# visinf/style-seqcvae

Hardware: AMD Instinct MI355X
Metric: captions/sec (train step) (higher is better)
Workload: dtype f32; 1 GPU; C2 train step: fwd+bwd+allreduce+clip+SGD, B=64/GPU, R=36, F=2048, L=20 (T=21), Z=128, V=10000, E=1000, H=1200, A=768, SENTIMENT_VAE=1; global_batch=64, parallelism=dp1

## Files before the change

include/ssc.h:

```cpp
#ifndef SSC_H
#define SSC_H

#include <stddef.h>
#include <stdint.h>

#ifdef __cplusplus
extern "C" {
#endif

#define SSC_OK 0
#define SSC_EINVAL (-1)
#define SSC_EALIGN (-2)
#define SSC_EHIP (-3)
#define SSC_EWORKSPACE (-4)

#define SSC_MAX_SEG 6

int ssc_version(void);
int ssc_last_hip_error(void);
const char* ssc_arch(void);

typedef struct {
  const float* A; const float* B;
  int lda, ldb, K;
  const void* A16; const void* B16;
  int lda16, ldb16;
} ssc_gemm_seg;

typedef struct {
  ssc_gemm_seg seg[SSC_MAX_SEG];
  int nseg;
  int M, N;
  int a_kc, b_kc;
  float* C; int ldc;
  const float* bias;
  int accumulate;
  int splits;
  float* workspace; size_t workspace_floats;
  const int* m_count; const int* a_rows; const int* c_rows;
  const int* k_count; const int* ka_rows; const int* kb_rows;
  const float* a_scale; const float* b_scale;
  float* topk_part;
} ssc_gemm_desc;

int ssc_pow2_scale(const float* x, size_t rows, int cols, size_t ld, int target_log2, float* out, int combine, float* scratch,
                   void* stream);

int ssc_split_f16(const float* x, int rows, int K, int ldx, const float* scale, void* out, int ldo, const int* row_list,
                  const int* row_count, void* stream);

int ssc_gemm(const ssc_gemm_desc* d, void* stream);

int ssc_gemm_dw_group(const ssc_gemm_desc* const* d, int n, void* stream);

int ssc_set_gemm_mode(int mode);
int ssc_gemm_auto_splits(int M, int N, int ksteps);

int ssc_feat_prep(const float* feats, int B, int R, int F, float* mask, float* avg, void* stream);

int ssc_prep_tokens(const int64_t* caps, int B, int L, int pad, int boundary, int64_t* tokens_tm, float* w_tm,
                    float* nvalid, void* stream);

int ssc_embed_gather(const float* table, int ldt, const int64_t* ids, int n, int E, float* out, int ldo, void* stream);
int ssc_embed_scatter_add(float* dtable, int ldt, const int64_t* ids, int n, int E, const float* d, int ldd, int pad,
                          void* stream);

typedef struct {
  int B, H;
  const float* slabs; int nslab; size_t slab_stride;
  const float* add0; int ld_add0;
  const float* add1; int ld_add1; int rows_per_add1;
  const float* b_ih; const float* b_hh;
  const float* sent; const float* wcol; int ldwcol;
  const float* c_prev; int ld_cprev;
  float* gates_out;
  float* c_out; int ld_cout;
  float* h_out; int ld_hout;
  const int64_t* add0_rows;
  const int* slab_rows;
  const float* slabs2; int nslab2; size_t slab2_stride; const int* slab2_rows;
  const int* c_prev_rows;
  const int* rows; const int* row_count;
  void* h_planes; int ld_hplanes; const float* planes_scale;
} ssc_lstm_fwd_desc;
int ssc_lstm_fwd(const ssc_lstm_fwd_desc* d, void* stream);
int ssc_lstm_fwd_z(const ssc_lstm_fwd_desc* d, const float* z, int ldz, const float* wz, int ldwz, int Z, void* stream);
int ssc_lstm_fwd_p(const ssc_lstm_fwd_desc* d, const float* wp, int ldwp, int NP, float* pout, void* stream);
int ssc_lstm_fwd_img(const ssc_lstm_fwd_desc* d, const float* alpha, int ldalpha, const float* P, int R, int rows_per_image,
                     void* stream);

typedef struct {
  int B, H;
  const float* dh; int ld_dh;
  const float* dh2; int ld_dh2;
  const float* dc_in; int ld_dcin;
  const float* gates;
  const float* c_prev; int ld_cprev;
  const float* c_new; int ld_cnew;
  float* dG;
  float* dc_prev; int ld_dcprev;
  float* dgsum;
  const float* slabsA; int nA; size_t strideA;
  const float* slabsB; int nB; size_t strideB;
} ssc_lstm_bwd_desc;
int ssc_lstm_bwd(const ssc_lstm_bwd_desc* d, void* stream);
int ssc_lstm_bwd_x(const ssc_lstm_bwd_desc* d, const float* x, int ldx, const float* w, int ldw, int K, void* stream);

int ssc_attn_logits(const float* q, int ldq, const float* pv, const float* wa, int G, int R, int A, int rows_per_image,
                    float* logits, void* stream);
int ssc_attn_fwd(const float* q, int ldq, const float* pv, const float* wa, const float* mask, const float* feats,
                 int G, int R, int A, int F, int rows_per_image, float* logits, float* alpha, float* att, int ldatt,
                 void* stream);

int ssc_attn_weights(const float* q, int ldq, const float* pv, const float* wa, const float* mask, int G, int R, int A,
                     int rows_per_image, float* logits, float* alpha, void* stream);

int ssc_attn_pool(const float* alpha, const float* x, int G, int R, int D, int rows_per_image, float* out, int ldo,
                  void* stream);
int ssc_attn_fwd_pool(const float* q, int ldq, const float* pv, const float* wa, const float* mask, const float* feats,
                      int G, int R, int A, int F, int rows_per_image, float* logits, float* alpha, float* att, int ldatt,
                      const float* obj, int D, float* pool, int ldpool, void* stream);

int ssc_attn_bwd(const float* datt, int lddatt, const float* q, int ldq, const float* pv, const float* wa,
                 const float* alpha, const float* feats, int G, int R, int A, int F, float* dq, int lddq,
                 float* dpv_acc, float* dwa_acc, float* scratch_dalpha, void* stream);
int ssc_attn_bwd_pool(const float* datt, int lddatt, const float* q, int ldq, const float* pv, const float* wa,
                      const float* alpha, const float* feats, int G, int R, int A, int F, float* dq, int lddq,
                      float* dpv_acc, float* dwa_acc, float* scratch_dalpha, const float* obj, int D, const float* dpool_a,
                      int lddpa, int Da, const float* dpool_b, int lddpb, void* stream);

typedef struct {
  int B, Z;
  const float* mulv; int ldmulv; int nslab; size_t slab_stride;
  const float* bmu; const float* blv;
  const float* eps; int ldeps;
  int kld_mode;
  const float* sent; float pm_scale; float prior_var;
  const float* w;
  float* mu; float* lv; float* z; int ldz;
  float* kld_acc;
  const float* pm; int ldpm;
} ssc_latent_fwd_desc;
int ssc_latent_fwd(const ssc_latent_fwd_desc* d, void* stream);

// ... 472 lines not shown
```

style-seqcvae_amd/csrc/gemm.hip:

```cpp
#include <stdio.h>
#include <stdlib.h>
#include <string.h>

#include "ssc_common.h"
#include "ssc_debug.h"

typedef float f32x16 __attribute__((ext_vector_type(16)));

namespace {

constexpr int BM = 64, BN = 64, BK = 32;
constexpr int KC_LD = BK + 4;

struct KSeg {
  const float* A;
  const float* B;
  int lda, ldb, K, nsteps;
  int avec, bvec;
  const float* A16;
  const float* B16;
  int lda16, ldb16;
};

struct KArgs {
  KSeg seg[SSC_MAX_SEG];
  int nseg;
  int M, N;
  float* out;
  int ldo;
  size_t slab_stride;
  const float* bias;
  int accumulate;
  int steps_total, steps_per_split;
  const int* mcount;
  const int* arows;
  const int* crows;
  const int* kcount;
  const int* karows;
  const int* kbrows;
  int tile_gm;
  int store_wt;
  int member;
  float* topk;
  const float* a_scale;
  const float* b_scale;
};

__device__ __forceinline__ void tile_order(int lin, int gx, int gy, int gm, int& bx, int& by) {
  const int total = gx * gy;
  const int q = total >> 3, rem = total & 7;
  const int xcd = lin & 7, slot = lin >> 3;
  const int nl = xcd * q + (xcd < rem ? xcd : rem) + slot;
  if (gm <= 1 || gy <= 1) {
    by = nl / gx;
    bx = nl - by * gx;
    return;
  }
  const int group_sz = gm * gx;
  const int g = nl / group_sz;
  const int first_row = g * gm;
  const int rows = min(gy - first_row, gm);
  const int r = nl - g * group_sz;
  bx = r / rows;
  by = first_row + (r - bx * rows);
}

template <bool KC, int ROWS, bool VEC>
__device__ __forceinline__ unsigned load_tile(float (&r)[ROWS / 8], const float* __restrict__ base, int ld, int rows, int K,
                                              int row0, int k0, int tid) {
  constexpr int NV = ROWS / 32;
  unsigned okm = 0;
  if constexpr (KC && VEC) {
#pragma unroll
    for (int u = 0; u < NV; ++u) {
      int idx = tid + 256 * u;
      int row = idx >> 3, kq = idx & 7;
      int grow = min(row0 + row, rows - 1), k = k0 + 4 * kq;
      float4 v = *reinterpret_cast<const float4*>(base + (size_t)grow * ld + min(k, K - 4));
      okm |= (k < K ? 1u : 0u) << u;
      r[4 * u] = v.x; r[4 * u + 1] = v.y; r[4 * u + 2] = v.z; r[4 * u + 3] = v.w;
    }
  } else if constexpr (KC && !VEC) {
#pragma unroll
    for (int u = 0; u < 4 * NV; ++u) {
      int idx = tid + 256 * u;
// ... 765 lines not shown
      SSC_X3B_MFMA(0, 2)
      SSC_X3B_MFMA(1, 1)
      SSC_X3B_MFMA(1, 0)
      SSC_X3B_MFMA(0, 1)
      SSC_X3B_MFMA(0, 0)
#undef SSC_X3B_MFMA
    }
  };

  for (int s = s_lo; s < s_hi; ++s) {
    compute();
    wait_loads();
    __syncthreads();
    if (s + 1 < s_hi) put_planes();
    advance();
    issue_loads();
    __syncthreads();
  }
  wait_loads();

  float* out = a.out + (size_t)z * a.slab_stride;
#pragma unroll
  for (int ni = 0; ni < 2; ++ni) {
    const int col = n0 + wn * 64 + ni * 32 + l31;
    if (col >= a.N) continue;
    const float bv = (a.bias != nullptr) ? a.bias[col] : 0.f;
#pragma unroll
    for (int mi = 0; mi < 2; ++mi) {
      const int rbase = m0 + wm * 64 + mi * 32 + 4 * half;
      int rr[16];
#pragma unroll
      for (int r = 0; r < 16; ++r) {
        rr[r] = min(rbase + (r & 3) + 8 * (r >> 2), Meff - 1);
        if (a.crows) rr[r] = a.crows[rr[r]];
      }
      float old[16];
      if (a.accumulate) {
#pragma unroll
        for (int r = 0; r < 16; ++r) old[r] = out[(size_t)rr[r] * a.ldo + col];
      } else {
#pragma unroll
        for (int r = 0; r < 16; ++r) old[r] = 0.f;
      }
#pragma unroll
      for (int r = 0; r < 16; ++r) {
        if (rbase + (r & 3) + 8 * (r >> 2) < Meff) out[(size_t)rr[r] * a.ldo + col] = acc[mi][ni][r] + bv + old[r];
      }
    }
  }
}


#ifdef SSC_X3W_STAMP
__device__ unsigned long long* g_stamp_ptr = nullptr;
__device__ int g_stamp_wg = -1;
#define SSC_STAMP(i)                                                                                  \
  do {                                                                                                \
    if (stamp_on && lane == 0 && (i) < 124) stamp_lds[(i)] = __builtin_readcyclecounter();           \
  } while (0)
constexpr int X3W_STAMP_BYTES = 2048;
#else
#define SSC_STAMP(i) do {} while (0)
constexpr int X3W_STAMP_BYTES = 0;
#endif
#ifdef SSC_X3W_AUDIT
constexpr int SSC_AUDIT_MEMBERS = 20;
__device__ long long g_audit[SSC_AUDIT_MEMBERS][SSC_MAX_SEG][2][2];
#define SSC_AUDIT_TOUCH(member, seg, op, off)                                       \
  do {                                                                              \
    atomicMin(&g_audit[(member)][(seg)][(op)][0], (long long)(off));                \
    atomicMax(&g_audit[(member)][(seg)][(op)][1], (long long)(off) + 16);           \
  } while (0)
#else
#define SSC_AUDIT_TOUCH(member, seg, op, off) do {} while (0)
#endif
template <int R> struct X3wPlane {
  static constexpr int MC_ROW_B = 2 * R + 64;
  static constexpr int KC_BYTES = R * PL_ROW_B, MC_BYTES = 32 * MC_ROW_B;
  static constexpr int BYTES = KC_BYTES > MC_BYTES ? KC_BYTES : MC_BYTES;
};
template <int TM, int TN> constexpr int x3w_lds_bytes() { return 2 * 3 * (X3wPlane<TM>::BYTES + X3wPlane<TN>::BYTES) + X3W_STAMP_BYTES; }
template <int TM, int TN> constexpr int x3w_lds_bytes_f16() { return 2 * 2 * (X3wPlane<TM>::BYTES + X3wPlane<TN>::BYTES) + X3W_STAMP_BYTES; }

template <bool A_KC, bool B_KC, bool KG, int TM, int TN, int PF, int NPW, bool F16 = false, class Args = KArgs>
__device__ __forceinline__ void x3w_body(const Args& a, const int blk_x, const int blk_y, const int blk_z, const int grid_x,
                                         const int grid_y, const int grid_z, const int thr) {
  static_assert((TM == 128 && TN == 128) || (TM == 64 && TN == 256), "unsupported tile");
  static_assert(PF == 1 || PF == 2, "prefetch depth");
  constexpr int UNR = 2;
  constexpr bool RL = TM == 128;
  static_assert(!KG || PF == 1, "the gather lists' own loads share the vector-memory counter");
  constexpr int NPL = F16 ? 2 : 3;
  constexpr int PLA = X3wPlane<TM>::BYTES, PLB = X3wPlane<TN>::BYTES, STAGE = NPL * (PLA + PLB);
  static_assert(TM * (TN + 4) * 4 <= 2 * STAGE, "the epilogue's C tile reuses the operand stages");
  constexpr int MCA = X3wPlane<TM>::MC_ROW_B, MCB = X3wPlane<TN>::MC_ROW_B;
  static_assert(NPW == 4 || NPW == 8, "producer waves");
  constexpr int NPT = 64 * NPW;
  constexpr int NTHR = 256 + NPT;
  constexpr int NA = TM * 8 / NPT, NB = TN * 8 / NPT;
  constexpr int QA = TM / 4, QB = TN / 4;
  auto kc_row = [&](int t, int u, int) __attribute__((always_inline)) -> int { return (t + NPT * u) >> 3; };
  extern __shared__ __attribute__((aligned(16))) unsigned char lds[];
  const int wave = thr >> 6;
  const bool producer = wave >= 4;
  const int tid = producer ? thr - 256 : thr;
  const int lane = tid & 63;
  int bx, by;
  const int Meff = (RL && a.mcount) ? min(a.M, *a.mcount) : a.M;
  const int gy_live = min(grid_y, (Meff + TM - 1) / TM);
  if (blk_y * grid_x + blk_x >= grid_x * gy_live) return;
  tile_order(blk_y * grid_x + blk_x, grid_x, gy_live, a.tile_gm, bx, by);
  const int n0 = bx * TN, m0 = by * TM, z = blk_z;
  if (m0 >= Meff) return;
  const int Kc = a.kcount ? max(0, min(a.seg[0].K, *a.kcount)) : 0;
  int steps_total = a.steps_total, steps_per_split = a.steps_per_split;
  if (a.kcount) {
    steps_total = (Kc + BK - 1) / BK;
    steps_per_split = (steps_total + grid_z - 1) / grid_z;
  }
  const int s_lo = z * steps_per_split;
  int s_hi = s_lo + steps_per_split;
  if (s_hi > steps_total) s_hi = steps_total;
  const int s_last = s_hi - 1;
  constexpr int CT_LD = TN + 4;
  float f16_sa = 1.f, f16_sb = 1.f;
  if constexpr (F16) {
    if (a.a_scale) f16_sa = *a.a_scale;
    if (a.b_scale) f16_sb = *a.b_scale;
  }
#ifdef SSC_X3W_STAMP
  const bool stamp_on = (int)blockIdx.x == g_stamp_wg && (wave == 0 || wave == 4);
  unsigned long long* stamp_lds = reinterpret_cast<unsigned long long*>(lds + 2 * STAGE) + (wave == 4 ? 0 : 128);
  if (stamp_on && lane == 0) { stamp_lds[126] = __builtin_readcyclecounter(); stamp_lds[127] = wall_clock64(); }
  const unsigned long long stamp_entry = wall_clock64();
#endif

  if (producer) {
    f32x4 ra[PF][NA], rb[PF][NB];
    unsigned oka[PF], okb[PF];
    bool fullk[PF];
    unsigned oa[NA], ob[NB];
    unsigned za[NA], zb[NB];
    int ia[2][NA], ib[2][NB];
    Cursor cur;
    int s_ld = s_lo;
    bool pa = false, pb = false;
    auto planes_of_segment = [&]() __attribute__((always_inline)) {
      if constexpr (F16) {
        const KSeg& sg = a.seg[cur.seg];
        pa = sg.A16 != nullptr; pb = sg.B16 != nullptr;
        if (pa) { cur.A = sg.A16; cur.lda = sg.lda16; }
        if (pb) { cur.B = sg.B16; cur.ldb = sg.ldb16; }
      }
    };
    auto base_ptrs = [&]() __attribute__((always_inline)) {
      const unsigned lda4 = (unsigned)cur.lda * 4u, ldb4 = (unsigned)cur.ldb * 4u;
#pragma unroll
      for (int u = 0; u < NA; ++u) {
        const int idx = tid + NPT * u;
        if constexpr (A_KC) {
          int r = min(m0 + kc_row(tid, u, NA), Meff - 1);
          if constexpr (RL) { if (a.arows) r = a.arows[r]; }
          za[u] = (unsigned)r * lda4;
          oa[u] = za[u] + 16u * (idx & 7);
        } else {
          za[u] = 4u * (unsigned)min(m0 + 4 * (idx % QA), Meff - 4);
// ... 326 lines not shown
        float mx = -INFINITY, v0 = -INFINITY, v1 = -INFINITY;
        int i0 = -1, i1 = -1;
        const float inv = F16 ? 1.0f / (f16_sa * f16_sb) : 1.0f;
        float x[32];
        const bool wide_b = a.bias && !(reinterpret_cast<uintptr_t>(a.bias) & 15) && n0 + TN <= a.N;
#pragma unroll
        for (int j = 0; j < 8; ++j) {
          const float4 c4 = *reinterpret_cast<const float4*>(&ct[row * CT_LD + part * 32 + 4 * j]);
          float4 b4 = make_float4(0.f, 0.f, 0.f, 0.f);
          const int gc = n0 + part * 32 + 4 * j;
          if (wide_b) b4 = *reinterpret_cast<const float4*>(a.bias + gc);
          else if (a.bias) { b4.x = gc < a.N ? a.bias[gc] : 0.f; b4.y = gc + 1 < a.N ? a.bias[gc + 1] : 0.f; b4.z = gc + 2 < a.N ? a.bias[gc + 2] : 0.f; b4.w = gc + 3 < a.N ? a.bias[gc + 3] : 0.f; }
          x[4 * j] = c4.x * inv + b4.x; x[4 * j + 1] = c4.y * inv + b4.y; x[4 * j + 2] = c4.z * inv + b4.z; x[4 * j + 3] = c4.w * inv + b4.w;
        }
#pragma unroll
        for (int j = 0; j < 32; ++j) {
          const int gcol = n0 + part * 32 + j;
          if (gcol < a.N) {
            mx = fmaxf(mx, x[j]);
            if (x[j] > v0) { v1 = v0; i1 = i0; v0 = x[j]; i0 = gcol; }
            else if (x[j] > v1) { v1 = x[j]; i1 = gcol; }
          }
        }
#pragma unroll
        for (int o = 1; o <= 2; o <<= 1) mx = fmaxf(mx, __shfl_xor(mx, o, 64));
        float se = 0.f;
#pragma unroll
        for (int j = 0; j < 32; ++j) {
          const int gcol = n0 + part * 32 + j;
          if (gcol < a.N) se += __builtin_amdgcn_exp2f((x[j] - mx) * 1.4426950408889634f);
        }
#pragma unroll
        for (int o = 1; o <= 2; o <<= 1) se += __shfl_xor(se, o, 64);
#pragma unroll
        for (int o = 1; o <= 2; o <<= 1) {
          const float w0 = __shfl_xor(v0, o, 64), w1 = __shfl_xor(v1, o, 64);
          const int j0 = __shfl_xor(i0, o, 64), j1 = __shfl_xor(i1, o, 64);
          auto before = [](float xa, int ia, float xb, int ib) { return ib < 0 || (ia >= 0 && (xa > xb || (xa == xb && ia < ib))); };
          float r0, r1; int k0, k1;
          if (before(v0, i0, w0, j0)) {
            r0 = v0; k0 = i0;
            if (before(v1, i1, w0, j0)) { r1 = v1; k1 = i1; } else { r1 = w0; k1 = j0; }
          } else {
            r0 = w0; k0 = j0;
            if (before(v0, i0, w1, j1)) { r1 = v0; k1 = i0; } else { r1 = w1; k1 = j1; }
          }
          v0 = r0; i0 = k0; v1 = r1; i1 = k1;
        }
        if (part == 0 && grow < Meff) {
          const int rr = (RL && a.crows) ? a.crows[grow] : grow;
          float* rec = a.topk + ((size_t)rr * ntn + bx) * 6;
          rec[0] = mx; rec[1] = se; rec[2] = v0; rec[3] = __int_as_float(i0); rec[4] = v1; rec[5] = __int_as_float(i1);
        }
      }
      return;
    }
  }
  {
    const float* ct = reinterpret_cast<const float*>(lds);
    float* out = a.out + (size_t)z * a.slab_stride;
    const bool wide = !(a.ldo & 3) && !(a.N & 3) && !(a.slab_stride & 3) && !(reinterpret_cast<uintptr_t>(a.out) & 15) &&
                      !(reinterpret_cast<uintptr_t>(a.bias) & 15);
    constexpr int CPR = TN / 4;
#pragma unroll
    for (int i = 0; i < (TM * CPR + NTHR - 1) / NTHR; ++i) {
      const int c = thr + NTHR * i;
      if (TM * CPR % NTHR != 0 && c >= TM * CPR) break;
      const int row = c / CPR, col = 4 * (c % CPR);
      const int grow = m0 + row, gcol = n0 + col;
      if (grow >= Meff || gcol >= a.N) continue;
      const int rr = (RL && a.crows) ? a.crows[grow] : grow;
      float4 v = *reinterpret_cast<const float4*>(&ct[row * CT_LD + col]);
      if constexpr (F16) { const float inv = 1.0f / (f16_sa * f16_sb); v.x *= inv; v.y *= inv; v.z *= inv; v.w *= inv; }
      float* dst = out + (size_t)rr * a.ldo + gcol;
      if (wide) {
        if (a.bias) { const float4 b4 = *reinterpret_cast<const float4*>(a.bias + gcol); v.x += b4.x; v.y += b4.y; v.z += b4.z; v.w += b4.w; }
        if (a.accumulate) { const float4 o4 = *reinterpret_cast<const float4*>(dst); v.x += o4.x; v.y += o4.y; v.z += o4.z; v.w += o4.w; }
        if (a.store_wt) {
          const f32x4 v4 = {v.x, v.y, v.z, v.w};
          asm volatile("global_store_dwordx4 %0, %1, off sc1" ::"v"(dst), "v"(v4) : "memory");
        } else {
          *reinterpret_cast<float4*>(dst) = v;
        }
      } else {
        const float e[4] = {v.x, v.y, v.z, v.w};
#pragma unroll
        for (int q = 0; q < 4; ++q) {
          if (gcol + q < a.N) dst[q] = e[q] + (a.bias ? a.bias[gcol + q] : 0.f) + (a.accumulate ? dst[q] : 0.f);
        }
      }
    }
  }
#ifdef SSC_X3W_STAMP
  if (stamp_on && lane == 0) { stamp_lds[124] = __builtin_readcyclecounter(); stamp_lds[125] = wall_clock64(); }
  __syncthreads();
  if ((int)blockIdx.x == g_stamp_wg && thr < 256 && g_stamp_ptr)
    g_stamp_ptr[thr] = reinterpret_cast<const unsigned long long*>(lds + 2 * STAGE)[thr];
  if (g_stamp_wg == -2 && thr == 0 && g_stamp_ptr && blockIdx.x < 1024) {
    g_stamp_ptr[2 * blockIdx.x] = stamp_entry;
    g_stamp_ptr[2 * blockIdx.x + 1] = wall_clock64();
  }
#endif
}


constexpr int SSC_GROUP_MAX = 6;
struct KGroup {
  KArgs a[SSC_GROUP_MAX];
  int n;
  int first[SSC_GROUP_MAX + 1];
  int gx[SSC_GROUP_MAX], gy[SSC_GROUP_MAX], gz[SSC_GROUP_MAX];
};
template <bool A_KC, bool B_KC, bool KG, int TM, int TN, int PF, int NPW, bool F16 = false>
__global__ __launch_bounds__(256 + 64 * NPW, (F16 && NPW == 4) ? 4 : 1) void gemm_x3w_kernel(const KGroup g) {
  const int w = blockIdx.x;
  int p = 0;
#pragma unroll
  for (int i = 1; i < SSC_GROUP_MAX; ++i)
    if (i < g.n && w >= g.first[i]) p = i;
  const int local = w - g.first[p];
  const int gx = g.gx[p], gy = g.gy[p], gz = g.gz[p];
  const int x = local % gx, yz = local / gx;
  x3w_body<A_KC, B_KC, KG, TM, TN, PF, NPW, F16>(g.a[p], x, yz % gy, yz / gy, gx, gy, gz, (int)threadIdx.x);
}

constexpr int SSC_DW_MAX = 20;
struct KTnMember {
  const float* A;
  const float* B;
  float* C;
  const int* kcount;
  const int* karows;
  const int* kbrows;
  int lda, ldb, ldc, M, N, K, accumulate;
  int first;
};
struct KTnList {
  KTnMember m[SSC_DW_MAX];
  int n, total;
  int tile_gm, store_wt;
};
struct KOneSeg {
  KSeg s;
  __device__ __forceinline__ const KSeg& operator[](int) const { return s; }
};
struct KTnArgs {
  KOneSeg seg;
  int nseg, M, N;
  float* out;
  int ldo;
  size_t slab_stride;
  const float* bias;
  int accumulate, steps_total, steps_per_split;
  const int *mcount, *arows, *crows, *kcount, *karows, *kbrows;
  int tile_gm, store_wt, member;
  float* topk;
  const float *a_scale, *b_scale;
};
template <int PF, int NPW>
__global__ __launch_bounds__(256 + 64 * NPW, 1) void gemm_x3w_kernel_tn_list(const KTnList g) {
  int p = 0;
  for (int t = blockIdx.x; t < g.total; t += gridDim.x) {
#pragma unroll 1
    while (p + 1 < g.n && t >= g.m[p + 1].first) ++p;
    const KTnMember& m = g.m[p];
    int thr = (int)threadIdx.x;
    asm volatile("" : "+v"(thr));
    __builtin_assume(thr >= 0 && thr < 256 + 64 * NPW);
    KTnArgs a;
    a.seg.s.A = m.A; a.seg.s.B = m.B; a.seg.s.lda = m.lda; a.seg.s.ldb = m.ldb; a.seg.s.K = m.K;
    a.seg.s.nsteps = (m.K + BK - 1) / BK; a.seg.s.avec = a.seg.s.bvec = 1;
    a.seg.s.A16 = a.seg.s.B16 = nullptr; a.seg.s.lda16 = a.seg.s.ldb16 = 0;
    a.nseg = 1; a.M = m.M; a.N = m.N;
    a.out = m.C; a.ldo = m.ldc; a.slab_stride = 0; a.bias = nullptr; a.accumulate = m.accumulate;
    a.steps_total = a.steps_per_split = a.seg.s.nsteps;
    a.mcount = a.arows = a.crows = nullptr;
    a.kcount = m.kcount; a.karows = m.karows; a.kbrows = m.kbrows;
    a.tile_gm = g.tile_gm; a.store_wt = g.store_wt; a.member = p;
    a.topk = nullptr; a.a_scale = a.b_scale = nullptr;
    const int gx = (m.N + 127) / 128, gy = (m.M + 127) / 128;
    const int local = t - m.first;
    x3w_body<false, false, true, 128, 128, PF, NPW>(a, local % gx, local / gx, 0, gx, gy, 1, thr);
    __syncthreads();
  }
}

__global__ void reduce_slabs_kernel(const float* __restrict__ slabs, int nslab, size_t slab_stride, int M, int N,
                                    float* __restrict__ C, int ldc, const float* __restrict__ bias, int accumulate,
                                    const int* __restrict__ mcount, const int* __restrict__ crows) {
  size_t i = (size_t)blockIdx.x * blockDim.x + threadIdx.x;
  if (mcount) M = min(M, *mcount);
  size_t total = (size_t)M * N;
  if (i >= total) return;
  int row = (int)(i / N), col = (int)(i % N);
  float v = 0.f;
  for (int s0 = 0; s0 < nslab; s0 += 8) {
    float t[8];
#pragma unroll
    for (int u = 0; u < 8; ++u) t[u] = slabs[(size_t)min(s0 + u, nslab - 1) * slab_stride + i];
#pragma unroll
    for (int u = 0; u < 8; ++u) v += (s0 + u < nslab) ? t[u] : 0.f;
  }
  if (bias) v += bias[col];
  if (crows) row = crows[row];
  float* p = C + (size_t)row * ldc + col;
  if (accumulate) v += *p;
  *p = v;
}

typedef void (*gemm_fn)(const KArgs);

struct ProfMember { int M, N, K, slot_m, slot_k; };
struct ProfRec {
  hipEvent_t e0, e1;
  int kind, M, N, K, splits;
  double bytes, flops;
  ProfMember mem[8];
  int nmem;
};
int* g_prof_counts = nullptr;
int g_prof_slots = 0;
constexpr int PROF_SLOTS = 8192;
inline int prof_count_slot(const int* dev_count, hipStream_t st) {
  if (!dev_count || !g_prof_counts || g_prof_slots >= PROF_SLOTS) return -1;
  const int slot = g_prof_slots++;
  g_prof_counts[slot] = -1;
  if (hipMemcpyAsync(&g_prof_counts[slot], dev_count, sizeof(int), hipMemcpyDeviceToHost, st) != hipSuccess) return -1;
  return slot;
}
inline void prof_desc(ProfRec* rec, const ssc_gemm_desc* d, hipStream_t st) {
  int K = 0;
  for (int i = 0; i < d->nseg; ++i) K += d->seg[i].K;
  if (rec->nmem < 8) {
    ProfMember& m = rec->mem[rec->nmem++];
    m.M = d->M; m.N = d->N; m.K = K;
    m.slot_m = prof_count_slot(d->m_count, st);
    m.slot_k = prof_count_slot(d->k_count, st);
  }
}
constexpr int PROF_MAX = 4096;
ProfRec* g_prof = nullptr;
int g_prof_n = 0;
bool g_prof_on = false;

int g_store_wt = ssc_env_int("SSC_STORE_WT", 1);
int g_tile_gm = ssc_env_int("SSC_TILE_GM", 8);
int build_args(const ssc_gemm_desc* d, KArgs& k) {
  if (!d || d->nseg < 1 || d->nseg > SSC_MAX_SEG || d->M <= 0 || d->N <= 0) return SSC_EINVAL;
  k.tile_gm = g_tile_gm;
  k.store_wt = g_store_wt;
  k.member = 0;
  k.nseg = d->nseg;
  k.M = d->M;
  k.N = d->N;
  k.mcount = d->m_count; k.arows = d->a_rows; k.crows = d->c_rows;
  k.kcount = d->k_count; k.karows = d->ka_rows; k.kbrows = d->kb_rows;
  k.a_scale = d->a_scale; k.b_scale = d->b_scale;
  k.topk = d->topk_part;
  k.steps_total = 0;
  for (int i = 0; i < d->nseg; ++i) {
    const ssc_gemm_seg& s = d->seg[i];
    if (!s.A || !s.B || s.K <= 0) return SSC_EINVAL;
// ... 384 lines not shown
  KGroup g;
  bool ok = n >= 2, any_wide = false;
  long work = 0;
  const bool mid = d[0] && d[0]->M > 64 && d[0]->M >= BIG_MIN_M;
  const int tw = mid ? 128 : 256;
  for (int i = 0; i < n && ok; ++i) {
    SSC_TRY(build_args(d[i], g.a[i]));
    const KArgs& k = g.a[i];
    const bool compact = k.mcount || k.arows || k.crows || k.kcount || k.karows || k.kbrows;
    const bool shape = mid ? g_x3b != 0 && g_x3b != 3 && d[i]->M >= BIG_MIN_M && d[i]->M < 512 && d[i]->M == d[0]->M
                           : x3w_skinny_layout(d[i]) && d[i]->M <= 64;
    ok = !compact && x3w_ok(d[i], k, num) && d[i]->a_kc && shape && d[i]->N >= 64 && d[i]->b_kc == d[0]->b_kc && regions[i];
    any_wide = any_wide || (mid ? big_tile(d[i]->M, d[i]->N) : d[i]->N >= X3W_MIN_N);
    work += (long)ssc_cdiv(d[i]->N, tw) * ssc_cdiv(d[i]->M, mid ? 128 : 64) * k.steps_total;
  }
  ok = ok && any_wide;
  if (!ok) {
    for (int i = 0; i < n; ++i) SSC_TRY(ssc_gemm_slabs_auto(d[i], regions[i], caps[i], &nslab[i], st));
    return SSC_OK;
  }
  int per = (int)((work + 255) / 256);
  if (per < 4) per = 4;
  for (;; ++per) {
    long wgs = 0;
    for (int i = 0; i < n; ++i) wgs += (long)ssc_cdiv(d[i]->N, tw) * ssc_cdiv(d[i]->M, mid ? 128 : 64) * ssc_cdiv(g.a[i].steps_total, per);
    if (wgs <= 256 || per >= 4096) break;
  }
  g.n = n;
  g.first[0] = 0;
  int Ksum = 0, Nmax = 0;
  for (int i = 0; i < n; ++i) {
    KArgs& k = g.a[i];
    k.member = i;
    const size_t mn = (size_t)d[i]->M * d[i]->N;
    int splits = ssc_cdiv(k.steps_total, per);
    const int cap = (int)(caps[i] / mn);
    if (cap < 1) return SSC_EWORKSPACE;
    if (splits > cap) splits = cap;
    const int p2 = ssc_cdiv(k.steps_total, splits);
    splits = ssc_cdiv(k.steps_total, p2);
    k.steps_per_split = p2;
    k.out = regions[i];
    k.ldo = d[i]->N;
    k.slab_stride = mn;
    k.bias = nullptr;
    k.accumulate = 0;
    k.crows = nullptr;
    g.gx[i] = ssc_cdiv(d[i]->N, tw);
    g.gy[i] = mid ? ssc_cdiv(d[i]->M, 128) : 1;
    g.gz[i] = splits;
    g.first[i + 1] = g.first[i] + g.gx[i] * g.gy[i] * splits;
    nslab[i] = splits;
    for (int s = 0; s < d[i]->nseg; ++s) Ksum += d[i]->seg[s].K;
    if (d[i]->N > Nmax) Nmax = d[i]->N;
  }
  for (int i = n; i < SSC_GROUP_MAX; ++i) { g.first[i + 1] = g.first[n]; g.gx[i] = 1; g.gy[i] = 1; g.gz[i] = 1; }
  ProfRec* rec = prof_open(d, n, d[0]->M, Nmax, Ksum, nslab[0], st);
  if (mid) return launch_x3w(x3w_big(true, d[0]->b_kc != 0, false), g, true, d[0]->b_kc != 0, "128x128 group", rec, st);
  return launch_x3w(x3w_skinny_form(d[0]->b_kc != 0), g, true, d[0]->b_kc != 0, "64x256 group", rec, st);
}

namespace {
int launch_tn_list(const ssc_gemm_desc* const* d, const KArgs* ka, int n, hipStream_t st) {
  SSC_TRY(x3w_prepare());
  int dev = 0;
  if (hipGetDevice(&dev) != hipSuccess) return SSC_EHIP;
  int ord[SSC_DW_MAX];
  for (int i = 0; i < n; ++i) ord[i] = i;
  for (int i = 1; i < n; ++i)
    for (int j = i; j > 0 && ka[ord[j]].steps_total > ka[ord[j - 1]].steps_total; --j) { const int t = ord[j]; ord[j] = ord[j - 1]; ord[j - 1] = t; }
  KTnList g;
  memset(&g, 0, sizeof(g));
  const ssc_gemm_desc* ds[SSC_DW_MAX];
  KArgs audit[SSC_DW_MAX];
  int first = 0;
  long MN = 0;
  for (int i = 0; i < n; ++i) {
    const ssc_gemm_desc* di = d[ord[i]];
    KTnMember& m = g.m[i];
    m.A = di->seg[0].A; m.B = di->seg[0].B; m.C = di->C;
    m.kcount = di->k_count; m.karows = di->ka_rows; m.kbrows = di->kb_rows;
    m.lda = di->seg[0].lda; m.ldb = di->seg[0].ldb; m.ldc = di->ldc;
    m.M = di->M; m.N = di->N; m.K = di->seg[0].K; m.accumulate = di->accumulate;
    m.first = first;
    first += ssc_cdiv(di->M, 128) * ssc_cdiv(di->N, 128);
    MN += (long)di->M * di->N;
    ds[i] = di;
    audit[i] = ka[ord[i]];
    audit[i].out = di->C; audit[i].ldo = di->ldc;
  }
  g.n = n; g.total = first;
  g.tile_gm = g_tile_gm; g.store_wt = g_store_wt;
  ProfRec* rec = prof_open(ds, n, (int)(MN / ds[0]->N), ds[0]->N, ds[0]->seg[0].K, 1, st);
  SSC_AUDIT_BEGIN();
  SSC_LAUNCH(g_tn_list_fn, dim3(first < g_cus[dev] ? first : g_cus[dev]), dim3(TN_LIST_THREADS), TN_LIST_LDS, st, g);
  SSC_AUDIT_END(audit, n, false, false, "128x128 TN list", st);
  (void)audit;
  prof_close(rec, st);
  SSC_CHECK_LAUNCH();
  return SSC_OK;
}
}
extern "C" int ssc_gemm_dw_group(const ssc_gemm_desc* const* d, int n, void* stream) {
  hipStream_t st = (hipStream_t)stream;
  constexpr int NMAX = 32;
  if (!d || n < 1 || n > NMAX) return SSC_EINVAL;
  const Num num = numerics();
  KArgs ka[NMAX];
  int cls[NMAX];
  for (int j = 0; j < n; ++j) {
    const ssc_gemm_desc* dj = d[j];
    KArgs& k = ka[j];
    SSC_TRY(build_args(dj, k));
    const bool kg = k.karows || k.kbrows;
    const bool ok = x3w_ok(dj, k, num) && k.nseg == 1 && !dj->a_kc && !dj->b_kc && dj->C && dj->ldc >= dj->N && !k.mcount &&
                    !k.arows && !k.crows && (kg ? (k.kcount && k.karows && k.kbrows && !dj->bias) : !k.kcount);
    cls[j] = !ok ? 0 : kg ? 2 : 1;
  }
  const ssc_gemm_desc* ld[SSC_DW_MAX];
  KArgs lk[SSC_DW_MAX];
  int ln = 0;
  for (int j = 0; j < n; ++j) {
    if (cls[j] != 2) continue;
    ld[ln] = d[j]; lk[ln] = ka[j];
    if (++ln == SSC_DW_MAX) { SSC_TRY(launch_tn_list(ld, lk, ln, st)); ln = 0; }
  }
  if (ln) SSC_TRY(launch_tn_list(ld, lk, ln, st));
  int i = 0;
  while (i < n) {
    if (cls[i] == 2) { ++i; continue; }
    int m = 0;
    while (cls[i] == 1 && i + m < n && cls[i + m] == 1 && m < SSC_GROUP_MAX) ++m;
    if (m >= 2) {
      KGroup g;
      g.n = m;
      g.first[0] = 0;
      long MN = 0;
      for (int q = 0; q < m; ++q) {
        const ssc_gemm_desc* dj = d[i + q];
        KArgs& k = g.a[q];
        k = ka[i + q];
        k.member = q;
        k.steps_per_split = k.steps_total;
        k.out = dj->C; k.ldo = dj->ldc; k.slab_stride = 0; k.bias = dj->bias; k.accumulate = dj->accumulate;
        g.gx[q] = ssc_cdiv(dj->N, 128); g.gy[q] = ssc_cdiv(dj->M, 128); g.gz[q] = 1;
        g.first[q + 1] = g.first[q] + g.gx[q] * g.gy[q];
        MN += (long)dj->M * dj->N;
      }
      for (int q = m; q < SSC_GROUP_MAX; ++q) { g.first[q + 1] = g.first[m]; g.gx[q] = g.gy[q] = g.gz[q] = 1; }
      ProfRec* rec = prof_open(d + i, m, (int)(MN / d[i]->N), d[i]->N, d[i + m - 1]->seg[0].K, 1, st);
      SSC_TRY(launch_x3w(x3w_big(false, false, false), g, false, false, "128x128 TN group", rec, st));
      i += m;
    } else {
      SSC_TRY(ssc_gemm(d[i], (void*)st));
      ++i;
    }
  }
  return SSC_OK;
}

namespace {
__global__ __launch_bounds__(256) void split_f16_kernel(const float* __restrict__ x, int rows, int K, int ldx, const float* __restrict__ scale,
                                                        unsigned* __restrict__ out, int ldo, const int* __restrict__ row_list,
                                                        const int* __restrict__ row_count) {
  const int kq = blockIdx.x * blockDim.x + threadIdx.x;
  const int kp4 = (K + BK - 1) / BK * (BK / 4);
  if (kq >= kp4) return;
  const float sc = scale ? *scale : 1.f;
  const int n = row_list ? min(rows, *row_count) : rows;
  const bool vec = !(ldx & 3) && ssc_aligned16_dev(x);
  const int k = 4 * kq;
  for (int i = blockIdx.y; i < n; i += gridDim.y) {
    const int r = row_list ? row_list[i] : i;
    const float* xr = x + (size_t)r * ldx;
    f32x4 v;
    if (k + 4 <= K && vec) v = *reinterpret_cast<const f32x4*>(xr + k);
    else
#pragma unroll
      for (int j = 0; j < 4; ++j) v[j] = k + j < K ? xr[k + j] : 0.f;
    v = v * sc;
    u32x2 hi, lo;
    split4_f16(v, hi, lo);
    unsigned* o = out + (size_t)r * ldo + (kq >> 3) * 32 + (kq & 7) * 2;
    *reinterpret_cast<u32x2*>(o) = hi;
    *reinterpret_cast<u32x2*>(o + 16) = lo;
  }
}
}
extern "C" int ssc_split_f16(const float* x, int rows, int K, int ldx, const float* scale, void* out, int ldo, const int* row_list,
                             const int* row_count, void* stream) {
  const int kp = ssc_cdiv(K, BK) * BK;
  if (!x || !out || rows <= 0 || K <= 0 || ldx < K || ldo < kp || (ldo & 3) || !ssc_aligned16(out) || (row_list != nullptr) != (row_count != nullptr))
    return SSC_EINVAL;
  SSC_LAUNCH(split_f16_kernel, dim3(ssc_cdiv(kp / 4, 256), rows < 65535 ? rows : 65535), dim3(256), 0, (hipStream_t)stream, x, rows, K, ldx, scale,
             static_cast<unsigned*>(out), ldo, row_list, row_count);
  SSC_CHECK_LAUNCH();
  return SSC_OK;
}

extern "C" int ssc_gemm(const ssc_gemm_desc* d, void* stream) {
  hipStream_t st = (hipStream_t)stream;
  KArgs k;
  SSC_TRY(build_args(d, k));
  if (d->topk_part) {
    k.out = nullptr; k.ldo = d->N; k.slab_stride = 0; k.bias = d->bias; k.accumulate = 0;
    return launch(d, k, 1, st);
  }
  if (!d->C || d->ldc < d->N) return SSC_EINVAL;
  int splits = d->splits;
  if (splits <= 0) splits = ssc_gemm_auto_splits(d->M, d->N, k.steps_total);
  if (splits > k.steps_total) splits = k.steps_total;
  {
    int per = ssc_cdiv(k.steps_total, splits);
    splits = ssc_cdiv(k.steps_total, per);
  }
  if (splits > 1 && (!d->workspace || d->workspace_floats < (size_t)splits * d->M * d->N)) {
    if (d->splits > 1) return SSC_EWORKSPACE;
    splits = d->workspace ? (int)(d->workspace_floats / ((size_t)d->M * d->N)) : 1;
    if (splits < 1) splits = 1;
    int per = ssc_cdiv(k.steps_total, splits);
    splits = ssc_cdiv(k.steps_total, per);
  }
  if (splits == 1) {
    k.out = d->C;
    k.ldo = d->ldc;
    k.slab_stride = 0;
    k.bias = d->bias;
    k.accumulate = d->accumulate;
    return launch(d, k, 1, st);
  }
  k.out = d->workspace;
  k.ldo = d->N;
  k.slab_stride = (size_t)d->M * d->N;
  k.bias = nullptr;
  k.accumulate = 0;
  k.crows = nullptr;
  SSC_TRY(launch(d, k, splits, st));
  size_t total = (size_t)d->M * d->N;
  SSC_LAUNCH(reduce_slabs_kernel, dim3((unsigned)((total + 255) / 256)), dim3(256), 0, st, d->workspace, splits,
                     k.slab_stride, d->M, d->N, d->C, d->ldc, d->bias, d->accumulate, d->m_count, d->c_rows);
  SSC_CHECK_LAUNCH();
  return SSC_OK;
}

extern "C" int ssc_prof_enable(int on) {
  if (on && !g_prof) {
    g_prof = new ProfRec[PROF_MAX];
    for (int i = 0; i < PROF_MAX; ++i) {
      if (hipEventCreate(&g_prof[i].e0) != hipSuccess || hipEventCreate(&g_prof[i].e1) != hipSuccess) return SSC_EHIP;
    }
  }
  if (on && !g_prof_counts && hipHostMalloc((void**)&g_prof_counts, PROF_SLOTS * sizeof(int), hipHostMallocDefault) != hipSuccess) return SSC_EHIP;
  g_prof_on = on != 0;
  if (on) { g_prof_n = 0; g_prof_slots = 0; }
  return SSC_OK;
}

extern "C" int ssc_prof_collect(float* out, int max_records) {
  if (!out || !g_prof) return 0;
  if (hipDeviceSynchronize() != hipSuccess) return SSC_EHIP;
  int n = g_prof_n < max_records ? g_prof_n : max_records;
  for (int i = 0; i < n; ++i) {
    float ms = 0.f;
    (void)hipEventElapsedTime(&ms, g_prof[i].e0, g_prof[i].e1);
    float* o = out + (size_t)i * 8;
    g_prof[i].bytes = g_prof[i].flops = 0.0;
    for (int q = 0; q < g_prof[i].nmem; ++q) {
      const ProfMember& m = g_prof[i].mem[q];
      double M = m.M, K = m.K;
      if (m.slot_m >= 0 && g_prof_counts[m.slot_m] >= 0 && g_prof_counts[m.slot_m] < m.M) M = g_prof_counts[m.slot_m];
      if (m.slot_k >= 0 && g_prof_counts[m.slot_k] >= 0 && g_prof_counts[m.slot_k] < m.K) K = g_prof_counts[m.slot_k];
      g_prof[i].bytes += 4.0 * (K * m.N + M * K + M * m.N);
      g_prof[i].flops += 2.0 * M * m.N * K;
    }
    o[0] = (float)g_prof[i].kind; o[1] = (float)g_prof[i].M; o[2] = (float)g_prof[i].N; o[3] = (float)g_prof[i].K;
    o[4] = (float)g_prof[i].splits; o[5] = ms; o[6] = (float)g_prof[i].bytes; o[7] = (float)g_prof[i].flops;
  }
  g_prof_n = 0;
  g_prof_slots = 0;
  return n;
}

extern "C" int ssc_set_gemm_mode(int mode) {
  int prev = gemm_mode();
  if (mode == 0 || mode == 1) g_gemm_mode = mode;
  return prev;
// ... 48 lines not shown
```

style-seqcvae_amd/csrc/pointwise.hip:

```cpp
#include <algorithm>

#include "ssc_common.h"

thread_local int ssc_tls_hip_error = 0;

extern "C" int ssc_version(void) { return 4; }
extern "C" int ssc_last_hip_error(void) { return ssc_tls_hip_error; }
extern "C" const char* ssc_arch(void) { return "gfx950"; }

namespace {

__global__ void feat_mask_kernel(const float* __restrict__ feats, int BR, int F, float* __restrict__ mask) {
  int row = blockIdx.x * (blockDim.x >> 6) + (threadIdx.x >> 6);
  int lane = threadIdx.x & 63;
  if (row >= BR) return;
  const float* p = feats + (size_t)row * F;
  float s = 0.f;
  for (int f = lane; f < F; f += 64) s += fabsf(p[f]);
  s = ssc_wave_sum(s);
  if (lane == 0) mask[row] = s > 0.f ? 1.f : 0.f;
}

__global__ void feat_avg_kernel(const float* __restrict__ feats, const float* __restrict__ mask, int R, int F,
                                float* __restrict__ avg) {
  int b = blockIdx.y;
  int f = blockIdx.x * blockDim.x + threadIdx.x;
  if (f >= F) return;
  const float* p = feats + (size_t)b * R * F + f;
  const float* m = mask + (size_t)b * R;
  float s = 0.f, n = 0.f;
  for (int r = 0; r < R; ++r) {
    float mr = m[r];
    s += mr * p[(size_t)r * F];
    n += mr;
  }
  avg[(size_t)b * F + f] = s / fmaxf(n, 1e-8f);
}

__global__ void prep_tokens_kernel(const int64_t* __restrict__ caps, int B, int L, int pad, int boundary,
                                   int64_t* __restrict__ tok, float* __restrict__ w, float* __restrict__ nvalid) {
  int b = blockIdx.x * blockDim.x + threadIdx.x;
  if (b >= B) return;
  int n = 0;
  for (int j = 0; j < L; ++j) n += caps[(size_t)b * L + j] != pad;
  tok[b] = boundary;
  for (int j = 0; j < L; ++j) tok[(size_t)(1 + j) * B + b] = caps[(size_t)b * L + j];
  tok[(size_t)(L + 1) * B + b] = 0;
  tok[(size_t)(n + 1) * B + b] = boundary;
  float nv = 0.f;
  for (int t = 0; t <= L; ++t) {
    float wt = tok[(size_t)(t + 1) * B + b] != pad ? 1.f : 0.f;
    w[(size_t)t * B + b] = wt;
    nv += wt;
  }
  nvalid[b] = nv;
}

__global__ void embed_gather_kernel(const float* __restrict__ table, int ldt, const int64_t* __restrict__ ids, int n, int E,
                                    float* __restrict__ out, int ldo) {
  int i = blockIdx.y;
  int e = blockIdx.x * blockDim.x + threadIdx.x;
  if (e >= E) return;
  out[(size_t)i * ldo + e] = table[(size_t)ids[i] * ldt + e];
}

constexpr int kEmbedScatterThreads = 256;
constexpr int kEmbedScatterChunk = 4096;
constexpr int kEmbedScatterBatch = 8;
constexpr int kEmbedScatterRows = 32;
__global__ void __launch_bounds__(kEmbedScatterThreads) embed_scatter_kernel(float* __restrict__ dt, int ldt,
                                                                               const int64_t* __restrict__ ids, int n, int E,
                                                                               const float* __restrict__ d, int ldd, int pad) {
  __shared__ unsigned long long s_hit[kEmbedScatterChunk / SSC_WAVE];
  __shared__ int s_pos[kEmbedScatterChunk + kEmbedScatterRows];
  __shared__ int s_cnt;
  const int i = blockIdx.y;
  const int e = blockIdx.x * kEmbedScatterThreads + threadIdx.x;
  const int64_t id = ids[i];
  if (id == pad) return;
  constexpr int kSpan = kEmbedScatterBatch * kEmbedScatterThreads;
  bool earlier = false;
  for (int j0 = threadIdx.x; j0 < i; j0 += kSpan) {
    int64_t v[kEmbedScatterBatch];
#pragma unroll
    for (int u = 0; u < kEmbedScatterBatch; ++u) v[u] = ids[min(j0 + u * kEmbedScatterThreads, i - 1)];
#pragma unroll
    for (int u = 0; u < kEmbedScatterBatch; ++u) earlier |= j0 + u * kEmbedScatterThreads < i && v[u] == id;
  }
  if (__syncthreads_or(earlier)) return;
  const int lane = threadIdx.x % SSC_WAVE;
  for (int c0 = i; c0 < n; c0 += kEmbedScatterChunk) {
    const int cn = min(kEmbedScatterChunk, n - c0);
    for (int k0 = 0; k0 < cn; k0 += kSpan) {
      int64_t v[kEmbedScatterBatch];
#pragma unroll
      for (int u = 0; u < kEmbedScatterBatch; ++u) v[u] = ids[c0 + min(k0 + u * kEmbedScatterThreads + (int)threadIdx.x, cn - 1)];
#pragma unroll
      for (int u = 0; u < kEmbedScatterBatch; ++u) {
        const unsigned long long hit = __ballot(k0 + u * kEmbedScatterThreads + (int)threadIdx.x < cn && v[u] == id);
        if (lane == 0) s_hit[(k0 + u * kEmbedScatterThreads + threadIdx.x) / SSC_WAVE] = hit;
      }
    }
    __syncthreads();
    const int nw = (cn + SSC_WAVE - 1) / SSC_WAVE;
    if (threadIdx.x < SSC_WAVE) {
      const unsigned long long m0 = lane < nw ? s_hit[lane] : 0ull;
      const int c = __popcll(m0);
      int incl = c;
#pragma unroll
      for (int o = 1; o < SSC_WAVE; o <<= 1) {
        const int t = __shfl_up(incl, o, SSC_WAVE);
        if (lane >= o) incl += t;
      }
      int q = incl - c;
      for (unsigned long long m = m0; m; m &= m - 1) s_pos[q++] = lane * SSC_WAVE + __builtin_ctzll(m);
      if (lane == SSC_WAVE - 1) s_cnt = incl;
    }
    __syncthreads();
    const int cnt = s_cnt;
// ... 501 lines not shown
  }
  const float l = lse[row];
  const int tgt = (int)targets[row];
#pragma unroll 2
  for (int i = threadIdx.x; i < n4; i += 256) {
    float4 x = p4[i];
    const int v = head + (i << 2);
    x.x = (expf(x.x - l) - (v == tgt ? keep : 0.f) - eps_over_v) * coef;
    x.y = (expf(x.y - l) - (v + 1 == tgt ? keep : 0.f) - eps_over_v) * coef;
    x.z = (expf(x.z - l) - (v + 2 == tgt ? keep : 0.f) - eps_over_v) * coef;
    x.w = (expf(x.w - l) - (v + 3 == tgt ? keep : 0.f) - eps_over_v) * coef;
    p4[i] = x;
  }
  for (int k = threadIdx.x; k < ns; k += 256) {
    const int v = k < head ? k : tail + (k - head);
    p[v] = (expf(p[v] - l) - (v == tgt ? keep : 0.f) - eps_over_v) * coef;
  }
}

__global__ void log_softmax_kernel(const float* __restrict__ logits, int ldl, int V, float* __restrict__ out, int ldo) {
  __shared__ float sh[16];
  int row = blockIdx.x;
  const float* p = logits + (size_t)row * ldl;
  float* o = out + (size_t)row * ldo;
  float mx = -INFINITY;
  for (int v = threadIdx.x; v < V; v += blockDim.x) mx = fmaxf(mx, p[v]);
  mx = block_reduce(mx, sh, true);
  float s = 0.f;
  for (int v = threadIdx.x; v < V; v += blockDim.x) s += expf(p[v] - mx);
  s = block_reduce(s, sh, false);
  float l = mx + logf(s);
  for (int v = threadIdx.x; v < V; v += blockDim.x) o[v] = p[v] - l;
}

constexpr int COLSUM_CHUNKS = 64;
__global__ __launch_bounds__(256) void colsum_stage1_kernel(const float* __restrict__ X, int ldx, int rows, int N,
                                                            const float* __restrict__ wrow, float* __restrict__ part) {
  int n = blockIdx.x * 256 + threadIdx.x;
  int chunk = blockIdx.y;
  int per = (rows + COLSUM_CHUNKS - 1) / COLSUM_CHUNKS;
  int r0 = chunk * per, r1 = r0 + per < rows ? r0 + per : rows;
  if (n >= N) return;
  float s = 0.f;
  for (int r = r0; r < r1; r += 8) {
    float x[8];
#pragma unroll
    for (int u = 0; u < 8; ++u) {
      const int rr = min(r + u, r1 - 1);
      x[u] = X[(size_t)rr * ldx + n];
      if (wrow) x[u] *= wrow[rr];
    }
#pragma unroll
    for (int u = 0; u < 8; ++u) s += (r + u < r1) ? x[u] : 0.f;
  }
  part[(size_t)chunk * N + n] = s;
}
__global__ __launch_bounds__(256) void colsum_stage2_kernel(const float* __restrict__ part, int N, float* __restrict__ out,
                                                            int out_stride, float* __restrict__ out2, int accumulate) {
  __shared__ float sh[4][64];
  const int c = threadIdx.x & 63, q = threadIdx.x >> 6;
  const int n = blockIdx.x * 64 + c;
  float t = 0.f;
  if (n < N) {
    float x[COLSUM_CHUNKS / 4];
#pragma unroll
    for (int u = 0; u < COLSUM_CHUNKS / 4; ++u) x[u] = part[(size_t)(q * (COLSUM_CHUNKS / 4) + u) * N + n];
#pragma unroll
    for (int u = 0; u < COLSUM_CHUNKS / 4; ++u) t += x[u];
  }
  sh[q][c] = t;
  __syncthreads();
  if (q != 0 || n >= N) return;
  t = ((sh[0][c] + sh[1][c]) + sh[2][c]) + sh[3][c];
  float* o = out + (size_t)n * out_stride;
  *o = accumulate ? *o + t : t;
  if (out2) out2[n] = accumulate ? out2[n] + t : t;
}

__global__ void colsum_kernel(const float* __restrict__ X, int ldx, int rows, int N, const float* __restrict__ wrow,
                              float* __restrict__ out, int out_stride, float* __restrict__ out2, int accumulate) {
  int n = blockIdx.x * blockDim.x + threadIdx.x;
  if (n >= N) return;
  float s = 0.f;
  for (int r = 0; r < rows; ++r) {
    float x = X[(size_t)r * ldx + n];
    s += wrow ? wrow[r] * x : x;
  }
  float* o = out + (size_t)n * out_stride;
  *o = accumulate ? *o + s : s;
  if (out2) out2[n] = accumulate ? out2[n] + s : s;
}

__global__ void copy_strided_kernel(const float* __restrict__ src, size_t stride, int n, float* __restrict__ dst) {
  int i = blockIdx.x * blockDim.x + threadIdx.x;
  if (i < n) dst[i] = src[(size_t)i * stride];
}

__global__ void bias_tanh_kernel(float* __restrict__ x, int ldx, int N, const float* __restrict__ bias) {
  int r = blockIdx.y;
  int n = blockIdx.x * blockDim.x + threadIdx.x;
  if (n >= N) return;
  float* p = x + (size_t)r * ldx + n;
  *p = tanhf(*p + (bias ? bias[n] : 0.f));
}

__global__ void tanh_bwd_kernel(float* __restrict__ dy, int lddy, const float* __restrict__ y, int ldy, int N) {
  int r = blockIdx.y;
  int n = blockIdx.x * blockDim.x + threadIdx.x;
  if (n >= N) return;
  float yy = y[(size_t)r * ldy + n];
  dy[(size_t)r * lddy + n] *= (1.f - yy * yy);
}

__global__ void fill_kernel(float* __restrict__ p, size_t n, float v) {
  size_t i = (size_t)blockIdx.x * blockDim.x + threadIdx.x;
  size_t stride = (size_t)gridDim.x * blockDim.x;
  for (; i < n; i += stride) p[i] = v;
}

template <bool NT> __device__ __forceinline__ float stream_ld(const float* p) { return NT ? __builtin_nontemporal_load(p) : *p; }
template <bool NT> __device__ __forceinline__ void stream_st(float* p, float v) {
  if (NT) __builtin_nontemporal_store(v, p);
  else *p = v;
}
template <bool NT>
__global__ void sq_norm_partial_kernel(const float* __restrict__ g, size_t n, float* __restrict__ scratch) {
  __shared__ float sh[16];
  size_t i = (size_t)blockIdx.x * blockDim.x + threadIdx.x;
  size_t stride = (size_t)gridDim.x * blockDim.x;
  float s = 0.f;
  if (ssc_aligned16_dev(g)) {
    const size_t n4 = n >> 2;
    const ssc_f32x4* g4 = reinterpret_cast<const ssc_f32x4*>(g);
    for (size_t k = i; k < n4; k += stride) {
      const ssc_f32x4 v = NT ? __builtin_nontemporal_load(&g4[k]) : g4[k];
      s += v.x * v.x + v.y * v.y + v.z * v.z + v.w * v.w;
    }
    for (size_t k = (n4 << 2) + i; k < n; k += stride) { const float v = stream_ld<NT>(g + k); s += v * v; }
  } else {
    for (; i < n; i += stride) {
      float v = stream_ld<NT>(g + i);
      s += v * v;
    }
  }
  s = block_reduce(s, sh, false);
  if (threadIdx.x == 0) scratch[blockIdx.x] = s;
}

__global__ void sq_norm_final_kernel(const float* __restrict__ scratch, int nb, float* __restrict__ out) {
  __shared__ float sh[16];
  float s = 0.f;
  for (int i = threadIdx.x; i < nb; i += blockDim.x) s += scratch[i];
  s = block_reduce(s, sh, false);
  if (threadIdx.x == 0) *out = s;
}

template <bool NT>
__global__ void sgd_kernel(float* __restrict__ p, const float* __restrict__ g, float* __restrict__ buf, size_t n,
                           const float* __restrict__ sqnorm, float gscale, float max_norm, float lr, float momentum,
                           float wd, int first) {
  float norm = sqrtf(*sqnorm) * gscale;
  float coef = fminf(1.f, max_norm / (norm + 1e-6f)) * gscale;
  size_t i = (size_t)blockIdx.x * blockDim.x + threadIdx.x;
  size_t stride = (size_t)gridDim.x * blockDim.x;
  for (; i < n; i += stride) {
    float pv = stream_ld<NT>(p + i);
    float dd = stream_ld<NT>(g + i) * coef + wd * pv;
    float b = first ? dd : momentum * stream_ld<NT>(buf + i) + dd;
    stream_st<NT>(buf + i, b);
    stream_st<NT>(p + i, pv - lr * b);
  }
}

struct AdamArgs {
  float step_size;
  float rsqrt_bc2;
  float beta1, omb1, beta2, omb2, eps, wd;
  float decay;
};

template <bool DECOUPLED>
__device__ __forceinline__ void adam_elem(float& p, float g, float& m, float& v, float coef, const AdamArgs& a) {
  float d = g * coef;
  if (DECOUPLED) p = p * a.decay;
  else d = d + a.wd * p;
  m = a.beta1 * m + a.omb1 * d;
  v = a.beta2 * v + a.omb2 * d * d;
  p = p - a.step_size * (m / (sqrtf(v) * a.rsqrt_bc2 + a.eps));
}

template <bool DECOUPLED>
__global__ void adam_kernel(float* __restrict__ p, const float* __restrict__ g, float* __restrict__ m, float* __restrict__ v,
                            size_t n, size_t head, size_t n4, const float* __restrict__ sqnorm, float gscale, float max_norm,
                            AdamArgs a) {
  float norm = sqrtf(*sqnorm) * gscale;
  float coef = fminf(1.f, max_norm / (norm + 1e-6f)) * gscale;
  const size_t i = (size_t)blockIdx.x * blockDim.x + threadIdx.x;
  const size_t stride = (size_t)gridDim.x * blockDim.x;
  float4* p4 = reinterpret_cast<float4*>(p + head);
  const float4* g4 = reinterpret_cast<const float4*>(g + head);
  float4* m4 = reinterpret_cast<float4*>(m + head);
  float4* v4 = reinterpret_cast<float4*>(v + head);
  for (size_t k = i; k < n4; k += stride) {
    float4 pv = p4[k], gv = g4[k], mv = m4[k], vv = v4[k];
    adam_elem<DECOUPLED>(pv.x, gv.x, mv.x, vv.x, coef, a);
    adam_elem<DECOUPLED>(pv.y, gv.y, mv.y, vv.y, coef, a);
    adam_elem<DECOUPLED>(pv.z, gv.z, mv.z, vv.z, coef, a);
    adam_elem<DECOUPLED>(pv.w, gv.w, mv.w, vv.w, coef, a);
    p4[k] = pv;
    m4[k] = mv;
    v4[k] = vv;
  }
  const size_t tail = head + (n4 << 2);
  const size_t ns = head + (n - tail);
  for (size_t k = i; k < ns; k += stride) {
    const size_t e = k < head ? k : tail + (k - head);
    float pv = p[e], mv = m[e], vv = v[e];
    adam_elem<DECOUPLED>(pv, g[e], mv, vv, coef, a);
    p[e] = pv;
    m[e] = mv;
    v[e] = vv;
  }
}

inline hipStream_t S(void* s) { return (hipStream_t)s; }

}

extern "C" int ssc_feat_prep(const float* feats, int B, int R, int F, float* mask, float* avg, void* stream) {
  if (!feats || !mask || !avg || B <= 0 || R <= 0 || F <= 0) return SSC_EINVAL;
  int BR = B * R;
  SSC_LAUNCH(feat_mask_kernel, dim3(ssc_cdiv(BR, 4)), dim3(256), 0, S(stream), feats, BR, F, mask);
  SSC_CHECK_LAUNCH();
  SSC_LAUNCH(feat_avg_kernel, dim3(ssc_cdiv(F, 256), B), dim3(256), 0, S(stream), feats, mask, R, F, avg);
  SSC_CHECK_LAUNCH();
  return SSC_OK;
}

extern "C" int ssc_prep_tokens(const int64_t* caps, int B, int L, int pad, int boundary, int64_t* tokens_tm, float* w_tm,
                               float* nvalid, void* stream) {
  if (!caps || !tokens_tm || !w_tm || !nvalid || B <= 0 || L <= 0) return SSC_EINVAL;
  SSC_LAUNCH(prep_tokens_kernel, dim3(ssc_cdiv(B, 64)), dim3(64), 0, S(stream), caps, B, L, pad, boundary,
                     tokens_tm, w_tm, nvalid);
  SSC_CHECK_LAUNCH();
  return SSC_OK;
}

extern "C" int ssc_embed_gather(const float* table, int ldt, const int64_t* ids, int n, int E, float* out, int ldo,
                                void* stream) {
  if (!table || !ids || !out || n <= 0 || E <= 0 || ldt < E || ldo < E) return SSC_EINVAL;
  SSC_LAUNCH(embed_gather_kernel, dim3(ssc_cdiv(E, 256), n), dim3(256), 0, S(stream), table, ldt, ids, n, E, out,
                     ldo);
  SSC_CHECK_LAUNCH();
  return SSC_OK;
}

extern "C" int ssc_embed_scatter_add(float* dtable, int ldt, const int64_t* ids, int n, int E, const float* d, int ldd,
                                     int pad, void* stream) {
  if (!dtable || !ids || !d || n <= 0 || E <= 0 || ldt < E || ldd < E) return SSC_EINVAL;
  SSC_LAUNCH(embed_scatter_kernel, dim3(ssc_cdiv(E, kEmbedScatterThreads), n), dim3(kEmbedScatterThreads), 0, S(stream), dtable,
             ldt, ids, n, E, d, ldd, pad);
  SSC_CHECK_LAUNCH();
  return SSC_OK;
}

extern "C" int ssc_latent_fwd(const ssc_latent_fwd_desc* d, void* stream) {
  if (!d || d->B <= 0 || d->Z <= 0 || !d->mulv || d->nslab < 1 || !d->bmu || !d->blv || !d->eps || !d->w || !d->mu ||
      !d->lv || !d->z || !d->kld_acc)
    return SSC_EINVAL;
  const int zw = (d->Z + 63) / 64;
  if (d->nslab > 16 && (zw == 1 || zw == 2 || zw == 4))
    SSC_LAUNCH(latent_fwd_wide_kernel, dim3(d->B), dim3(256), 0, S(stream), *d);
  else
    SSC_LAUNCH(latent_fwd_kernel, dim3(ssc_cdiv(d->B, 4)), dim3(256), 0, S(stream), *d);
  SSC_CHECK_LAUNCH();
  return SSC_OK;
}

extern "C" int ssc_latent_prior_sample(const float* eps, int ldeps, const float* sent, float pm_scale, float prior_var,
                                       int G, int Z, float* z, int ldz, void* stream) {
  if (!eps || !z || G <= 0 || Z <= 0) return SSC_EINVAL;
  SSC_LAUNCH(latent_prior_sample_kernel, dim3(ssc_cdiv((Z + 3) & ~3, 64), G), dim3(64), 0, S(stream), eps, ldeps, sent,
                     pm_scale, sqrtf(prior_var), G, Z, z, ldz);
  SSC_CHECK_LAUNCH();
  return SSC_OK;
}

extern "C" int ssc_latent_prior_sample_pm(const float* eps, int ldeps, const float* pm, int ldpm, const float* pv, int ldpv,
                                          const float* sent, float pm_scale, float prior_var, int G, int Z, float* z, int ldz,
                                          void* stream) {
  if (!eps || !z || G <= 0 || Z <= 0 || ldeps < Z || (pm && ldpm < Z) || (pv && ldpv < Z) || ldz < Z) return SSC_EINVAL;
  SSC_LAUNCH(latent_prior_sample_pm_kernel, dim3(ssc_cdiv((Z + 3) & ~3, 64), G), dim3(64), 0, S(stream), eps, ldeps, pm, ldpm, pv, ldpv, sent,
             pm_scale, sqrtf(prior_var), G, Z, z, ldz);
  SSC_CHECK_LAUNCH();
  return SSC_OK;
}

extern "C" int ssc_latent_bwd(const ssc_latent_bwd_desc* d, void* stream) {
  if (!d || d->B <= 0 || d->Z <= 0 || !d->dz || !d->eps || !d->mu || !d->lv || !d->w || !d->gk || !d->dmulv)
    return SSC_EINVAL;
  SSC_LAUNCH(latent_bwd_kernel, dim3(ssc_cdiv(d->Z, 64), d->B), dim3(64), 0, S(stream), *d);
  SSC_CHECK_LAUNCH();
  return SSC_OK;
}

static bool free_bits_ok(const ssc_free_bits* fb) {
  if (!fb || !(fb->lambda >= 0.f) || !(fb->lambda <= 3.402823466e38f)) return false;
  return fb->lambda == 0.f || (fb->mode >= 1 && fb->mode <= 3);
}

extern "C" int ssc_latent_fwd_fb(const ssc_latent_fwd_desc* d, const ssc_free_bits* fb, void* stream) {
  if (!free_bits_ok(fb)) return SSC_EINVAL;
  if (fb->lambda == 0.f) return ssc_latent_fwd(d, stream);
  if (!d || d->B <= 0 || d->Z <= 0 || !d->mulv || d->nslab < 1 || !d->bmu || !d->blv || !d->eps || !d->w || !d->mu ||
      !d->lv || !d->z || !d->kld_acc)
    return SSC_EINVAL;
  if (!fb->kld_raw || (fb->mode == 2 && !fb->gate_step) || (fb->mode == 3 && (!fb->dim_acc || fb->lddim < d->Z))) return SSC_EINVAL;
// ... 279 lines not shown
```

style-seqcvae_amd/csrc/sequence.hip:

```cpp
#include <cstdlib>
#include <initializer_list>

#include "sample_draw.h"
#include "ssc_common.h"
#include "ssc_debug.h"

namespace {

inline size_t r4(size_t x) { return (x + 3) & ~(size_t)3; }

struct Layout {
  int B, R, L, T;
  int V, E, H, A, F, Z, S, tied;
  int Ep, Hp, Ap, Fp, Zp, Vp, H4, XW;
  int D, Dp, SC, NX;
  size_t wc_e, wc_d, pool, dpm;
  size_t total = 0;
  size_t act;
  size_t live;
  size_t tok, w, nvalid, sent_all, wcol_e, wcol_d, mask, avg, pv, emb, ga_static, ga_avg;
  size_t h1, c1, he, ce, hd, cd, gates_a, gates_e, gates_d, q, attn_logits, alpha, att, mu, lv, z, mulv;
  size_t slabs, slab_floats, logits, lse, proj;
  size_t nllw0, nll;
  size_t kld_raw, fb_kdim, fb_gdim, fb_gstep, fb_acc;
  size_t fed_ids, fed;
  size_t sl_q, sl_mulv, sl_gh1, sl_ghd, sl_ghd2, sl_ghe, sl_dqw, sl_dhe, sl_dz, small_floats, wsum_att, wsum_dec, wz;
  size_t sl_ga, sl_ge, sl_gd, gate_floats;
  size_t dhdv, dga, dge, dgd, dga_sum, g_h1, g_c1, g_he, g_ce, g_cd, dz, dmulv, dx, dalpha, dq, dpv, dwa, demb, dproj;

  size_t take(size_t n) {
    size_t o = total;
    total += (n + 63) & ~(size_t)63;
    return o;
  }
};

Layout make_layout(const ssc_model_cfg* c, int B, int R, int L) {
  Layout l;
  l.B = B; l.R = R; l.L = L; l.T = L + 1;
  l.V = c->V; l.E = c->E; l.H = c->H; l.A = c->A; l.F = c->F; l.Z = c->Z; l.S = c->S; l.tied = c->tied;
  l.Ep = (int)r4(l.E); l.Hp = (int)r4(l.H); l.Ap = (int)r4(l.A); l.Fp = (int)r4(l.F); l.Zp = (int)r4(l.Z);
  l.Vp = (int)r4(l.V); l.H4 = 4 * l.H;
  l.D = c->kld_mode == 2 ? c->Z : 0; l.Dp = (int)r4(l.D); l.SC = l.D ? c->S : 0;
  l.NX = l.D ? (int)r4(l.F + 2 * l.H + l.SC) : l.F + 2 * l.H;
  l.XW = (int)r4(l.NX);
  const size_t T = l.T, TB = T * B, T1B = (T + 1) * (size_t)B;
  l.tok = l.take(2 * (size_t)(L + 2) * B);
  l.w = l.take(TB);
  l.nvalid = l.take(B);
  l.act = l.take(TB + 4);
  l.live = l.take(TB + 4);
  l.sent_all = l.take(TB);
  l.wcol_e = l.take(l.H4); l.wcol_d = l.take(l.H4);
  l.mask = l.take((size_t)B * R);
  l.avg = l.take((size_t)B * l.Fp);
  l.pv = l.take((size_t)B * R * l.A);
  l.emb = l.take(TB * l.Ep);
  l.ga_static = l.take(TB * l.H4);
  l.ga_avg = l.take((size_t)B * l.H4);
  l.h1 = l.take(T1B * l.Hp); l.c1 = l.take(T1B * l.Hp);
  l.he = l.take(T1B * l.Hp); l.ce = l.take(T1B * l.Hp);
  l.hd = l.take(T1B * l.Hp); l.cd = l.take(T1B * l.Hp);
  l.gates_a = l.take(TB * l.H4); l.gates_e = l.take(TB * l.H4); l.gates_d = l.take(TB * l.H4);
  l.q = l.take(TB * l.Ap);
  l.attn_logits = l.take((size_t)B * R);
  l.alpha = l.take(TB * R);
  l.att = l.take(TB * l.Fp);
  l.mu = l.take(TB * l.Zp); l.lv = l.take(TB * l.Zp); l.z = l.take(TB * l.Zp);
  l.mulv = l.take((size_t)B * 2 * l.Z);
  size_t skinny = (size_t)33 * B * l.H4;
  size_t full = (size_t)16 * 1024 * 1024;
  l.slab_floats = skinny > full ? skinny : full;
  l.slabs = l.take(l.slab_floats);
  {
    size_t w = (size_t)(l.Hp > l.Ap ? l.Hp : l.Ap);
    if ((size_t)2 * l.Z > w) w = (size_t)2 * l.Z;
    l.small_floats = (size_t)40 * B * w;
    l.sl_q = l.take(l.small_floats); l.sl_mulv = l.take(l.small_floats);
    l.sl_gh1 = l.take(l.small_floats); l.sl_ghd = l.take(l.small_floats); l.sl_ghe = l.take(l.small_floats);
    l.sl_ghd2 = l.take(l.small_floats);
    l.sl_dqw = l.take(l.small_floats); l.sl_dhe = l.take(l.small_floats); l.sl_dz = l.take(l.small_floats);
  }
  l.gate_floats = (size_t)34 * B * l.H4;
  l.sl_ga = l.take(l.gate_floats); l.sl_ge = l.take(l.gate_floats); l.sl_gd = l.take(l.gate_floats);
  l.wsum_att = l.take((size_t)l.H4 * l.Hp);
  l.wsum_dec = l.take((size_t)l.H4 * l.Hp);
  l.wz = l.take((size_t)l.H4 * l.Zp);
  l.wc_e = l.take((size_t)l.H4 * l.Dp); l.wc_d = l.take((size_t)l.H4 * l.Dp);
  l.pool = l.take(TB * l.Dp); l.dpm = l.take((size_t)B * l.Dp);
  l.logits = l.take(TB * l.Vp);
  l.lse = l.take(2 * TB);
  l.proj = l.take(l.tied ? TB * l.Ep : 0);
  l.dhdv = l.take(TB * l.Hp);
  l.dga = l.take(TB * l.H4); l.dge = l.take(TB * l.H4); l.dgd = l.take(TB * l.H4);
  l.dga_sum = l.take((size_t)B * l.H4);
  l.g_h1 = l.take((size_t)B * l.Hp); l.g_c1 = l.take((size_t)B * l.Hp);
  l.g_he = l.take((size_t)B * l.Hp); l.g_ce = l.take((size_t)B * l.Hp);
  l.g_cd = l.take((size_t)B * l.Hp);
  l.dz = l.take((size_t)B * l.Zp);
  l.dmulv = l.take(TB * 2 * l.Z);
  l.dx = l.take((size_t)B * l.XW);
  l.dalpha = l.take((size_t)B * R);
  l.dq = l.take(TB * l.Ap);
  l.dpv = l.take((size_t)B * R * l.A);
  l.dwa = l.take((size_t)B * l.A);
  l.demb = l.take(TB * l.Ep);
  l.dproj = l.take(l.tied ? TB * l.Ep : 0);
  l.nllw0 = l.take(TB);
  l.nll = l.take(B);
  l.kld_raw = l.take(B);
  l.fb_kdim = l.take(l.Z); l.fb_gdim = l.take(l.Z);
  l.fb_gstep = l.take(TB);
  l.fb_acc = l.take((size_t)B * l.Zp);
  l.fed_ids = l.take(2 * TB);
  l.fed = l.take(TB);
  return l;
}

struct Seg {
  const float* A; int lda;
  const float* B; int ldb;
  int K;
};

struct Ctx {
  hipStream_t st;
  float* slabs;
  size_t slab_floats;
  const int* act_count = nullptr;
  const int* act_rows = nullptr;
  const int* live_count = nullptr;
  const int* live_rows = nullptr;
};

void fill_desc(ssc_gemm_desc& d, bool a_kc, bool b_kc, std::initializer_list<Seg> segs, int M, int N) {
  d = ssc_gemm_desc{};
  int i = 0;
  for (const Seg& s : segs) {
    if (s.K <= 0) continue;
    d.seg[i].A = s.A; d.seg[i].lda = s.lda; d.seg[i].B = s.B; d.seg[i].ldb = s.ldb; d.seg[i].K = s.K;
    ++i;
  }
  d.nseg = i;
  d.M = M; d.N = N;
  d.a_kc = a_kc; d.b_kc = b_kc;
}

int gemm(const Ctx& c, bool a_kc, bool b_kc, std::initializer_list<Seg> segs, int M, int N, float* C, int ldc,
         const float* bias = nullptr, int accumulate = 0) {
  ssc_gemm_desc d;
  fill_desc(d, a_kc, b_kc, segs, M, N);
  d.C = C; d.ldc = ldc; d.bias = bias; d.accumulate = accumulate;
  d.splits = 0;
  d.workspace = c.slabs; d.workspace_floats = c.slab_floats;
  return ssc_gemm(&d, c.st);
}

int gemm_rows(const Ctx& c, bool b_kc, std::initializer_list<Seg> segs, int M, int N, float* C, int ldc, const float* bias = nullptr,
              bool live = false) {
  ssc_gemm_desc d;
  fill_desc(d, true, b_kc, segs, M, N);
  d.C = C; d.ldc = ldc; d.bias = bias; d.accumulate = 0;
  d.splits = 0;
  d.workspace = c.slabs; d.workspace_floats = c.slab_floats;
  if (c.act_rows) {
    const int* cnt = live ? c.live_count : c.act_count;
    const int* rows = live ? c.live_rows : c.act_rows;
    d.m_count = cnt; d.a_rows = rows; d.c_rows = rows;
    const int rc = ssc_gemm(&d, c.st);
    if (rc != SSC_EALIGN && rc != SSC_EINVAL) return rc;
    d.m_count = d.a_rows = d.c_rows = nullptr;
  }
  return ssc_gemm(&d, c.st);
}
struct DwBatch {
  static constexpr int MAX = 24;
  ssc_gemm_desc d[MAX];
  int n = 0;
};
int queue_dw(const Ctx& c, DwBatch& q, const float* A, int lda, const float* Bm, int ldb, int K, int M, int N, float* C, int ldc) {
  if (q.n >= DwBatch::MAX) return SSC_EINVAL;
  ssc_gemm_desc& d = q.d[q.n++];
  fill_desc(d, false, false, {{A, lda, Bm, ldb, K}}, M, N);
  d.C = C; d.ldc = ldc;
  d.splits = 0;
  d.workspace = c.slabs; d.workspace_floats = c.slab_floats;
  if (c.live_rows) { d.k_count = c.live_count; d.ka_rows = c.live_rows; d.kb_rows = c.live_rows; }
  return SSC_OK;
}
int flush_dw(const Ctx& c, DwBatch& q) {
  if (!q.n) return SSC_OK;
  const ssc_gemm_desc* dp[DwBatch::MAX];
  for (int i = 0; i < q.n; ++i) dp[i] = &q.d[i];
  for (int i = 0; i < q.n; ++i) {
    ssc_gemm_desc& d = q.d[i];
    const bool al = ssc_aligned16(d.seg[0].A) && ssc_aligned16(d.seg[0].B) && !(d.seg[0].lda & 3) && !(d.seg[0].ldb & 3) && !(d.M & 3) && !(d.N & 3);
    if (!al) d.k_count = d.ka_rows = d.kb_rows = nullptr;
  }
  int rc = ssc_gemm_dw_group(dp, q.n, c.st);
  if (rc == SSC_EINVAL || rc == SSC_EALIGN) {
    for (int i = 0; i < q.n; ++i) q.d[i].k_count = q.d[i].ka_rows = q.d[i].kb_rows = nullptr;
    rc = ssc_gemm_dw_group(dp, q.n, c.st);
  }
  q.n = 0;
  return rc;
}
__global__ __launch_bounds__(1024) void build_active_rows_kernel(const float* __restrict__ w, int n, int B, int* __restrict__ act,
                                                                 int* __restrict__ live) {
  __shared__ int part[1024];
  const int tid = threadIdx.x;
  const bool suffix = blockIdx.x == 1;
  int* out = suffix ? live : act;
  auto flag = [&](int i) -> bool {
    if (!suffix) return w[i] != 0.f;
    for (int r = i; r < n; r += B)
      if (w[r] != 0.f) return true;
    return false;
  };
  const int per = (n + 1023) / 1024;
  const int lo = min(tid * per, n), hi = min(lo + per, n);
  int cnt = 0;
  for (int i = lo; i < hi; ++i) cnt += flag(i);
  part[tid] = cnt;
  __syncthreads();
  for (int off = 1; off < 1024; off <<= 1) {
    const int v = tid >= off ? part[tid - off] : 0;
    __syncthreads();
    part[tid] += v;
    __syncthreads();
  }
  int pos = part[tid] - cnt;
  for (int i = lo; i < hi; ++i)
    if (flag(i)) out[4 + pos++] = i;
  if (tid == 1023) out[0] = part[1023];
  for (int i = part[1023] + tid; i < n; i += 1024) out[4 + i] = 0;
}

int gemm_to_slabs(const Ctx& c, float* region, size_t cap, bool a_kc, bool b_kc, std::initializer_list<Seg> segs, int M,
                  int N, int* nslab) {
  ssc_gemm_desc d;
  fill_desc(d, a_kc, b_kc, segs, M, N);
  return ssc_gemm_slabs_auto(&d, region, cap, nslab, c.st);
}
int gemm_to_slabs(const Ctx& c, std::initializer_list<Seg> segs, int M, int N, int* nslab) {
  return gemm_to_slabs(c, c.slabs, c.slab_floats, true, true, segs, M, N, nslab);
}

__global__ void add2d_kernel(const float* __restrict__ a, int lda, const float* __restrict__ b, int ldb, int cols,
                             float* __restrict__ o, int ldo) {
  int r = blockIdx.y, x = blockIdx.x * blockDim.x + threadIdx.x;
  if (x < cols) o[(size_t)r * ldo + x] = a[(size_t)r * lda + x] + b[(size_t)r * ldb + x];
}
int add2d(const float* a, int lda, const float* b, int ldb, int rows, int cols, float* o, int ldo, hipStream_t st) {
  SSC_LAUNCH(add2d_kernel, dim3(ssc_cdiv(cols, 256), rows), dim3(256), 0, st, a, lda, b, ldb, cols, o, ldo);
  SSC_CHECK_LAUNCH();
  return SSC_OK;
}
struct ViewArgs {
  const float *att_ih, *att_hh, *dec_ih, *dec_hh, *dec_z, *enc_s, *dec_s;
  int ld_att_ih, ld_att_hh, ld_dec_ih, ld_dec_hh, ld_enc_ih;
  int H, Hp, Z, Zp, S, D, Dp, SC;
  float *wsum_att, *wsum_dec, *wz, *wcol_e, *wcol_d, *wc_e, *wc_d;
};
__global__ void weight_views_kernel(const ViewArgs a) {
  const int n = blockIdx.x, tid = threadIdx.x;
  for (int k = tid; k < a.H; k += blockDim.x) {
    a.wsum_att[(size_t)n * a.Hp + k] = a.att_ih[(size_t)n * a.ld_att_ih + k] + a.att_hh[(size_t)n * a.ld_att_hh + k];
    a.wsum_dec[(size_t)n * a.Hp + k] = a.dec_ih[(size_t)n * a.ld_dec_ih + k] + a.dec_hh[(size_t)n * a.ld_dec_hh + k];
  }
  for (int k = tid; k < a.Zp; k += blockDim.x) a.wz[(size_t)n * a.Zp + k] = k < a.Z ? a.dec_z[(size_t)n * a.ld_dec_ih + k] : 0.f;
  if (a.S == 1 && !a.D && tid == 0) {
    a.wcol_e[n] = a.enc_s[(size_t)n * a.ld_enc_ih];
    a.wcol_d[n] = a.dec_s[(size_t)n * a.ld_dec_ih];
  }
  for (int k = tid; k < a.Dp; k += blockDim.x) {
    a.wc_e[(size_t)n * a.Dp + k] = k < a.SC ? a.enc_s[(size_t)n * a.ld_enc_ih + k] : 0.f;
    a.wc_d[(size_t)n * a.Dp + k] = k < a.SC ? a.dec_s[(size_t)n * a.ld_dec_ih + k] : 0.f;
  }
}
int prepare_weight_views(const Layout& l, const ssc_params* p, float* W, hipStream_t st) {
  const int E = l.E, F = l.F, H = l.H, S = l.S;
  ViewArgs a;
  a.att_ih = p->att_w_ih + E + F; a.att_hh = p->att_w_hh; a.dec_ih = p->dec_w_ih + F + H; a.dec_hh = p->dec_w_hh;
  a.dec_z = p->dec_w_ih + F + 2 * H + S; a.enc_s = p->enc_w_ih + F + 2 * H; a.dec_s = p->dec_w_ih + F + 2 * H;
  a.ld_att_ih = p->ld_att_w_ih; a.ld_att_hh = p->ld_att_w_hh; a.ld_dec_ih = p->ld_dec_w_ih; a.ld_dec_hh = p->ld_dec_w_hh;
  a.ld_enc_ih = p->ld_enc_w_ih;
  a.H = H; a.Hp = l.Hp; a.Z = l.Z; a.Zp = l.Zp; a.S = S; a.D = l.D; a.Dp = l.Dp; a.SC = l.SC;
  a.wc_e = W + l.wc_e; a.wc_d = W + l.wc_d;
  a.wsum_att = W + l.wsum_att; a.wsum_dec = W + l.wsum_dec; a.wz = W + l.wz; a.wcol_e = W + l.wcol_e; a.wcol_d = W + l.wcol_d;
  SSC_LAUNCH(weight_views_kernel, dim3(l.H4), dim3(256), 0, st, a);
  SSC_CHECK_LAUNCH();
  return SSC_OK;
}

struct FillList {
  static constexpr int MAX = 16;
  float* p[MAX];
  size_t n[MAX];
  int count = 0;
  void add(float* ptr, size_t len) { if (len && count < MAX) { p[count] = ptr; n[count] = len; ++count; } }
};
__global__ void fill_many_kernel(const FillList f, float v) {
  float* p = f.p[blockIdx.y];
  const size_t n = f.n[blockIdx.y];
  for (size_t i = (size_t)blockIdx.x * blockDim.x + threadIdx.x; i < n; i += (size_t)gridDim.x * blockDim.x) p[i] = v;
}
int fill_many(const FillList& f, float v, hipStream_t st) {
  if (f.count == 0) return SSC_OK;
  SSC_LAUNCH(fill_many_kernel, dim3(256, f.count), dim3(256), 0, st, f, v);
  SSC_CHECK_LAUNCH();
  return SSC_OK;
}

int check_cfg(const ssc_model_cfg* c, const ssc_params* p, const ssc_batch* b) {
  if (!c || !p || !b) return SSC_EINVAL;
  if (c->V <= 1 || c->E <= 0 || c->H <= 0 || c->A <= 0 || c->F <= 0 || c->Z <= 0) return SSC_EINVAL;
  if (c->kld_mode < 0 || c->kld_mode > 2) return SSC_EINVAL;
  if (!(c->label_smoothing >= 0.f && c->label_smoothing < 1.f)) return SSC_EINVAL;
  if (c->kld_mode == 2 ? ((c->S != 1 && c->S != c->Z) || c->pm_scale != 0.f || !b->obj_atts) : (c->S != 0 && c->S != 1)) return SSC_EINVAL;
  if (b->B <= 0 || b->R <= 0 || b->L <= 0 || b->R > 256) return SSC_EINVAL;
  if (!b->feats || !b->caps || !b->eps) return SSC_EINVAL;
  if (((c->S == 1 && c->kld_mode != 2) || c->pm_scale != 0.f) && !b->sentiment) return SSC_EINVAL;
  if (!p->emb || !p->att_w_ih || !p->att_w_hh || !p->att_b_ih || !p->att_b_hh || !p->wq || !p->wv || !p->wa ||
      !p->enc_w_ih || !p->enc_w_hh || !p->enc_b_ih || !p->enc_b_hh || !p->dec_w_ih || !p->dec_w_hh || !p->dec_b_ih ||
      !p->dec_b_hh || !p->fc_mean_w || !p->fc_mean_b || !p->fc_lv_w || !p->fc_lv_b)
    return SSC_EINVAL;
  if (c->tied ? (!p->proj_w || !p->proj_b) : (!p->out_w || !p->out_b)) return SSC_EINVAL;
  return SSC_OK;
}

int check_free_bits(float free_bits, int mode) {
  if (!(free_bits >= 0.f) || !(free_bits <= 3.402823466e38f)) return SSC_EINVAL;
  if (free_bits > 0.f && (mode < 1 || mode > 3)) return SSC_EINVAL;
  return SSC_OK;
}

struct LoopProf {
  hipEvent_t e[4];
  bool created = false, on = false, fwd = false, bwd = false;
} g_loop;

}

extern "C" int ssc_prof_loop_enable(int on) {
  if (on && !g_loop.created) {
    for (hipEvent_t& e : g_loop.e)
      if (hipEventCreate(&e) != hipSuccess) return SSC_EHIP;
    g_loop.created = true;
  }
  g_loop.on = on != 0;
  g_loop.fwd = g_loop.bwd = false;
  return SSC_OK;
}
extern "C" int ssc_prof_loop_ms(float* fwd_loop_ms, float* bwd_loop_ms) {
  if (!fwd_loop_ms || !bwd_loop_ms) return SSC_EINVAL;
  *fwd_loop_ms = *bwd_loop_ms = -1.f;
  if (g_loop.fwd) {
    if (hipEventSynchronize(g_loop.e[1]) != hipSuccess || hipEventElapsedTime(fwd_loop_ms, g_loop.e[0], g_loop.e[1]) != hipSuccess) return SSC_EHIP;
  }
  if (g_loop.bwd) {
    if (hipEventSynchronize(g_loop.e[3]) != hipSuccess || hipEventElapsedTime(bwd_loop_ms, g_loop.e[2], g_loop.e[3]) != hipSuccess) return SSC_EHIP;
  }
  return SSC_OK;
}

extern "C" size_t ssc_train_workspace_bytes(const ssc_model_cfg* cfg, int B, int R, int L) {
  if (!cfg || B <= 0 || R <= 0 || L <= 0) return 0;
  return make_layout(cfg, B, R, L).total * sizeof(float);
}

extern "C" void* ssc_train_workspace_view(const ssc_model_cfg* cfg, int B, int R, int L, void* workspace, int which,
                                          int* ld) {
  if (!cfg || !workspace) return nullptr;
  Layout l = make_layout(cfg, B, R, L);
  float* w = (float*)workspace;
  int dummy;
  if (!ld) ld = &dummy;
  switch (which) {
    case 0: *ld = l.Hp; return w + l.h1;
    case 1: *ld = l.Hp; return w + l.c1;
    case 2: *ld = l.Hp; return w + l.he;
    case 3: *ld = l.Hp; return w + l.ce;
    case 4: *ld = l.Hp; return w + l.hd;
    case 5: *ld = l.Hp; return w + l.cd;
    case 6: *ld = l.R; return w + l.alpha;
    case 7: *ld = l.Zp; return w + l.mu;
    case 8: *ld = l.Zp; return w + l.lv;
    case 9: *ld = l.Vp; return w + l.logits;
    case 10: *ld = l.B; return w + l.tok;
    case 11: *ld = l.Fp; return w + l.att;
    case 12: *ld = l.B; return w + l.nll;
    default: return nullptr;
  }
}

extern "C" void* ssc_train_free_bits_view(const ssc_model_cfg* cfg, int B, int R, int L, void* workspace, int which, int* ld) {
  if (!cfg || !workspace || B <= 0 || R <= 0 || L <= 0) return nullptr;
  const Layout l = make_layout(cfg, B, R, L);
  float* w = (float*)workspace;
  int dummy;
  if (!ld) ld = &dummy;
  switch (which) {
    case 0: *ld = l.B; return w + l.kld_raw;
    case 1: *ld = l.Z; return w + l.fb_kdim;
    case 2: *ld = l.B; return w + l.fb_gstep;
    case 3: *ld = l.Z; return w + l.fb_gdim;
    default: return nullptr;
  }
}

extern "C" void* ssc_train_sched_view(const ssc_model_cfg* cfg, int B, int R, int L, void* workspace, int which, int* ld) {
  if (!cfg || !workspace || B <= 0 || R <= 0 || L <= 0) return nullptr;
  const Layout l = make_layout(cfg, B, R, L);
  float* w = (float*)workspace;
  int dummy;
  if (!ld) ld = &dummy;
  switch (which) {
    case 13: *ld = l.B; return w + l.fed_ids;
    case 14: *ld = l.B; return w + l.fed;
    default: return nullptr;
  }
}

extern "C" int ssc_train_fwd(const ssc_model_cfg* cfg, const ssc_params* p, const ssc_batch* bt, void* workspace,
                             size_t workspace_bytes, float* loss, float* kld, void* stream) {
  return ssc_train_fwd_fb(cfg, p, bt, workspace, workspace_bytes, loss, kld, 0.f, 0, stream);
}

static int train_fwd_impl(const ssc_model_cfg* cfg, const ssc_params* p, const ssc_batch* bt, void* workspace, size_t workspace_bytes,
                          float* loss, float* kld, float free_bits, int free_bits_mode, const ssc_sched_sampling* ss, void* stream) {
  SscGemmModeScope mode_scope(cfg);
  SSC_TRY(check_cfg(cfg, p, bt));
  SSC_TRY(check_free_bits(free_bits, free_bits_mode));
  if (ss && (!(ss->prob >= 0.f && ss->prob <= 1.f) || !sampler_ok(&ss->sampler, cfg->V))) return SSC_EINVAL;
  if (!workspace || !loss || !kld) return SSC_EINVAL;
  const bool ss_on = ss && ss->prob > 0.f;
  if (!ssc_aligned16(workspace)) return SSC_EALIGN;
  const Layout l = make_layout(cfg, bt->B, bt->R, bt->L);
  if (workspace_bytes < l.total * sizeof(float)) return SSC_EWORKSPACE;
  float* W = (float*)workspace;
  hipStream_t st = (hipStream_t)stream;
  Ctx c{st, W + l.slabs, l.slab_floats};
  const int B = l.B, R = l.R, T = l.T, E = l.E, H = l.H, A = l.A, F = l.F, Z = l.Z, S = l.S, V = l.V, H4 = l.H4;
  const int TB = T * B;
  int64_t* tok = (int64_t*)(W + l.tok);
  const size_t sH = (size_t)B * l.Hp;
  const bool fb_on = free_bits > 0.f;

  SSC_TRY(ssc_prep_tokens(bt->caps, B, l.L, cfg->pad, cfg->boundary, tok, W + l.w, W + l.nvalid, st));
  int* act = (int*)(W + l.act);
  int* live = (int*)(W + l.live);
  SSC_LAUNCH(build_active_rows_kernel, dim3(2), dim3(1024), 0, st, W + l.w, TB, B, act, live);
  SSC_CHECK_LAUNCH();
  c.act_count = act; c.act_rows = act + 4;
  c.live_count = live; c.live_rows = live + 4;
  SSC_TRY(ssc_feat_prep(bt->feats, B, R, F, W + l.mask, W + l.avg, st));
  SSC_TRY(gemm(c, true, true, {{bt->feats, F, p->wv, p->ld_wv, F}}, B * R, A, W + l.pv, A));
  const int hoisted = ss_on ? B : TB;
  SSC_TRY(ssc_embed_gather(p->emb, p->ld_emb, tok, hoisted, E, W + l.emb, l.Ep, st));
  SSC_TRY(gemm(c, true, true, {{W + l.emb, l.Ep, p->att_w_ih, p->ld_att_w_ih, E}}, hoisted, H4, W + l.ga_static, H4));
  int64_t* fed_ids = (int64_t*)(W + l.fed_ids);
  if (ss_on && hipMemcpyAsync(fed_ids, tok, (size_t)B * sizeof(int64_t), hipMemcpyDeviceToDevice, st) != hipSuccess) return SSC_EHIP;
  SSC_TRY(gemm(c, true, true, {{W + l.avg, F, p->att_w_ih + E, p->ld_att_w_ih, F}}, B, H4, W + l.ga_avg, H4));
  {
    FillList f;
    for (size_t off : {l.h1, l.c1, l.he, l.ce, l.hd, l.cd}) f.add(W + off, sH);
    f.add(kld, (size_t)B);
    if (fb_on) {
      f.add(W + l.kld_raw, (size_t)B);
      if (free_bits_mode == 3) f.add(W + l.fb_acc, (size_t)B * l.Zp);
    }
    if (l.Zp != Z) {
      f.add(W + l.z, (size_t)TB * l.Zp); f.add(W + l.mu, (size_t)TB * l.Zp); f.add(W + l.lv, (size_t)TB * l.Zp);
    }
    if (cfg->tied) f.add(W + l.proj, (size_t)TB * l.Ep);
    if (ss_on) f.add(W + l.fed, (size_t)B);
    SSC_TRY(fill_many(f, 0.f, st));
  }
  SSC_TRY(prepare_weight_views(l, p, W, st));
  const bool fc_adjacent = (p->fc_lv_w == p->fc_mean_w + (size_t)Z * p->ld_fc_mean_w) && p->ld_fc_lv_w == p->ld_fc_mean_w;

  auto head_step = [&](int t) -> int {
    const float* hd_t = W + l.hd + (size_t)(t + 1) * sH;
    float* logits_t = W + l.logits + (size_t)t * B * l.Vp;
    if (cfg->tied) {
      float* proj_t = W + l.proj + (size_t)t * B * l.Ep;
      SSC_TRY(gemm(c, true, true, {{hd_t, l.Hp, p->proj_w, p->ld_proj_w, H}}, B, E, proj_t, l.Ep));
      SSC_TRY(ssc_bias_tanh(proj_t, l.Ep, B, E, p->proj_b, st));
      return gemm(c, true, true, {{proj_t, l.Ep, p->emb, p->ld_emb, E}}, B, V, logits_t, l.Vp);
    }
    return gemm(c, true, true, {{hd_t, l.Hp, p->out_w, p->ld_out_w, H}}, B, V, logits_t, l.Vp, p->out_b);
  };

  if (g_loop.on) { (void)hipEventRecord(g_loop.e[0], st); }
  for (int t = 0; t < T; ++t) {
    if (ss_on && t > 0) {
      SSC_TRY(head_step(t - 1));
      float* emb_t = W + l.emb + (size_t)t * B * l.Ep;
      SSC_TRY(ssc_sched_mix_rows(W + l.logits + (size_t)(t - 1) * B * l.Vp, l.Vp, B, V, tok + (size_t)t * B, W + l.w + (size_t)(t - 1) * B,
                                 W + l.w + (size_t)t * B, p->emb, p->ld_emb, E, t, ss, fed_ids + (size_t)t * B, W + l.fed + (size_t)t * B,
                                 emb_t, l.Ep, st));
      SSC_TRY(gemm(c, true, true, {{emb_t, l.Ep, p->att_w_ih, p->ld_att_w_ih, E}}, B, H4, W + l.ga_static + (size_t)t * B * H4, H4));
    }
    float* h1p = W + l.h1 + t * sH; float* h1n = h1p + sH;
    float* c1p = W + l.c1 + t * sH; float* c1n = c1p + sH;
    float* hep = W + l.he + t * sH; float* hen = hep + sH;
    float* cep = W + l.ce + t * sH; float* cen = cep + sH;
    float* hdp = W + l.hd + t * sH; float* hdn = hdp + sH;
    float* cdp = W + l.cd + t * sH; float* cdn = cdp + sH;
    float* att = W + l.att + (size_t)t * B * l.Fp;
    float* qt = W + l.q + (size_t)t * B * l.Ap;
    float* zt = W + l.z + (size_t)t * B * l.Zp;
    float* poolt = l.D ? W + l.pool + (size_t)t * B * l.Dp : nullptr;
    int ns = 0;
    const size_t sG = (size_t)B * H4;
    int n_ga = 0, n_ge_r = 0, n_gd_r = 0, n_ge_a = 0, n_gd_a = 0;

    if (t > 0) {
      const float* wr = p->att_w_ih + E + F;
      ssc_gemm_desc d3[3];
      fill_desc(d3[0], true, true, {{h1p, l.Hp, W + l.wsum_att, l.Hp, H}, {hdp, l.Hp, wr + H, p->ld_att_w_ih, H}}, B, H4);
      fill_desc(d3[1], true, true, {{hdp, l.Hp, p->enc_w_ih + F + H, p->ld_enc_w_ih, H}, {hep, l.Hp, p->enc_w_hh, p->ld_enc_w_hh, H}}, B, H4);
      fill_desc(d3[2], true, true, {{hdp, l.Hp, W + l.wsum_dec, l.Hp, H}}, B, H4);
      const ssc_gemm_desc* dp[3] = {&d3[0], &d3[1], &d3[2]};
      float* regions[3] = {W + l.sl_ga, W + l.sl_ge, W + l.sl_gd};
      const size_t caps[3] = {l.gate_floats, l.gate_floats / 2, l.gate_floats / 2};
      int ns3[3] = {0, 0, 0};
      SSC_TRY(ssc_gemm_slabs_group(dp, 3, regions, caps, ns3, st));
      n_ga = ns3[0]; n_ge_r = ns3[1]; n_gd_r = ns3[2];
    }
    {
      ssc_lstm_fwd_desc d{};
      d.B = B; d.H = H;
      if (n_ga > 0) { d.slabs = W + l.sl_ga; d.nslab = n_ga; d.slab_stride = sG; }
      d.add0 = W + l.ga_static + (size_t)t * B * H4; d.ld_add0 = H4;
      d.add1 = W + l.ga_avg; d.ld_add1 = H4; d.rows_per_add1 = 1;
// ... 347 lines not shown
        SSC_TRY(gemm_to_slabs(c, W + l.sl_dhe, l.small_floats, true, false,
                              {{dmulv, 2 * Z, p->fc_mean_w, p->ld_fc_mean_w, Z}, {dmulv + Z, 2 * Z, p->fc_lv_w, p->ld_fc_lv_w, Z}}, B, H,
                              &ns));
        d.slabsB = W + l.sl_dhe; d.nB = ns; d.strideB = sBH;
        SSC_TRY(ssc_lstm_bwd(&d, st));
      }
    }
    {
      ssc_gemm_desc d2[2];
      fill_desc(d2[0], true, false, {{dge, H4, p->enc_w_ih, p->ld_enc_w_ih, H4}}, B, NX);
      fill_desc(d2[1], true, false, {{dge, H4, p->enc_w_hh, p->ld_enc_w_hh, H4}}, B, H);
      const ssc_gemm_desc* dp[2] = {&d2[0], &d2[1]};
      float* regions[2] = {c.slabs + (size_t)n_dxd * sBX, W + l.sl_ghe};
      const size_t caps[2] = {c.slab_floats - (size_t)n_dxd * sBX, l.small_floats};
      int ns2[2] = {0, 0};
      SSC_TRY(ssc_gemm_slabs_group(dp, t > 0 ? 2 : 1, regions, caps, ns2, st));
      n_dxe = ns2[0]; n_ghe = ns2[1];
    }
    SSC_TRY(ssc_reduce_slabs(c.slabs, n_dxd + n_dxe, sBX, B, NX, dx, XW, nullptr, 0, st));
    SSC_TRY(ssc_attn_bwd_pool(dx, XW, W + l.q + (size_t)t * B * l.Ap, l.Ap, W + l.pv, p->wa, W + l.alpha + (size_t)t * B * R,
                              bt->feats, B, R, A, F, dq, l.Ap, W + l.dpv, W + l.dwa, W + l.dalpha, l.D ? bt->obj_atts : nullptr, l.D,
                              dx + F + 2 * H, XW, l.SC, W + l.dpm, l.Dp, st));
    {
      ssc_lstm_bwd_desc d{};
      d.B = B; d.H = H;
      d.dh = dx + F; d.ld_dh = XW;
      d.slabsA = W + l.sl_gh1; d.nA = n_gh1; d.strideA = sBH;
      d.dc_in = W + l.g_c1; d.ld_dcin = l.Hp;
      d.gates = W + l.gates_a + (size_t)t * B * H4;
      d.c_prev = W + l.c1 + t * sH; d.ld_cprev = l.Hp;
      d.c_new = W + l.c1 + (t + 1) * sH; d.ld_cnew = l.Hp;
      d.dG = dga; d.dc_prev = W + l.g_c1; d.ld_dcprev = l.Hp;
      d.dgsum = W + l.dga_sum;
      const bool fused_q = A <= 768;
      if (fused_q) {
        SSC_TRY(ssc_lstm_bwd_x(&d, dq, l.Ap, p->wq, p->ld_wq, A, st));
      } else {
        SSC_TRY(gemm_to_slabs(c, W + l.sl_dqw, l.small_floats, true, false, {{dq, l.Ap, p->wq, p->ld_wq, A}}, B, H, &ns));
        d.slabsB = W + l.sl_dqw; d.nB = ns; d.strideB = sBH;
        SSC_TRY(ssc_lstm_bwd(&d, st));
      }
    }
    if (t > 0) {
      const float* wr = p->att_w_ih + E + F;
      ssc_gemm_desc d2[2];
      fill_desc(d2[0], true, false, {{dga, H4, W + l.wsum_att, l.Hp, H4}}, B, H);
      fill_desc(d2[1], true, false, {{dga, H4, wr + H, p->ld_att_w_ih, H4}}, B, H);
      const ssc_gemm_desc* dp[2] = {&d2[0], &d2[1]};
      float* regions[2] = {W + l.sl_gh1, W + l.sl_ghd};
      const size_t caps[2] = {l.small_floats, l.small_floats};
      int ns2[2] = {0, 0};
      SSC_TRY(ssc_gemm_slabs_group(dp, 2, regions, caps, ns2, st));
      n_gh1 = ns2[0]; n_ghd = ns2[1];
    }
  }

  if (g_loop.on) { (void)hipEventRecord(g_loop.e[3], st); g_loop.bwd = true; }

  if (S == 1 && !l.D) {
    SSC_LAUNCH(repeat_kernel, dim3(ssc_cdiv(TB, 256)), dim3(256), 0, st, bt->sentiment, B, T, W + l.sent_all);
    SSC_CHECK_LAUNCH();
  }
  }

  const int zcol = F + 2 * H + S;
  const float* dga = W + l.dga; const float* dge = W + l.dge; const float* dgd = W + l.dgd;
  const float* h1_prev = W + l.h1; const float* h1_new = W + l.h1 + sH;
  const float* hd_prev = W + l.hd; const float* he_prev = W + l.he; const float* he_new = W + l.he + sH;
  const float* att = W + l.att;
  if (phases & 64u) {
  if (g->emb && !cfg->tied) {
    SSC_TRY(ssc_fill(W + l.demb, (size_t)TB * l.Ep, 0.f, st));
    SSC_TRY(gemm_rows(c, false, {{dga, H4, p->att_w_ih, p->ld_att_w_ih, H4}}, TB, E, W + l.demb, l.Ep, nullptr, true));
    if (hipMemset2DAsync(g->emb, (size_t)g->ld_emb * sizeof(float), 0, (size_t)E * sizeof(float), V, st) != hipSuccess)
      return SSC_EHIP;
    SSC_TRY(ssc_embed_scatter_add(g->emb, g->ld_emb, fed_inputs ? (const int64_t*)(W + l.fed_ids) : tok, TB, E, W + l.demb, l.Ep,
                                  cfg->pad, st));
  }
  }
  auto queue_att = [&](DwBatch& q) -> int {
    if (g->att_w_ih) {
      float* gw = g->att_w_ih; int ld = g->ld_att_w_ih;
      SSC_TRY(queue_dw(c, q, dga, H4, W + l.emb, l.Ep, TB, H4, E, gw, ld));
      SSC_TRY(queue_dw(c, q, dga, H4, h1_prev, l.Hp, TB, H4, H, gw + E + F, ld));
      SSC_TRY(queue_dw(c, q, dga, H4, hd_prev, l.Hp, TB, H4, H, gw + E + F + H, ld));
    } else if (g->att_w_hh) {
      SSC_TRY(queue_dw(c, q, dga, H4, h1_prev, l.Hp, TB, H4, H, g->att_w_hh, g->ld_att_w_hh));
    }
    if (g->wq) SSC_TRY(queue_dw(c, q, W + l.dq, l.Ap, h1_new, l.Hp, TB, A, H, g->wq, g->ld_wq));
    return SSC_OK;
  };
  auto queue_enc = [&](DwBatch& q) -> int {
    if (g->enc_w_ih) {
      float* gw = g->enc_w_ih; int ld = g->ld_enc_w_ih;
      SSC_TRY(queue_dw(c, q, dge, H4, att, l.Fp, TB, H4, F, gw, ld));
      SSC_TRY(queue_dw(c, q, dge, H4, h1_new, l.Hp, TB, H4, H, gw + F, ld));
      SSC_TRY(queue_dw(c, q, dge, H4, hd_prev, l.Hp, TB, H4, H, gw + F + H, ld));
    }
    if (g->enc_w_hh) SSC_TRY(queue_dw(c, q, dge, H4, he_prev, l.Hp, TB, H4, H, g->enc_w_hh, g->ld_enc_w_hh));
    if (g->enc_w_ih && l.D) SSC_TRY(queue_dw(c, q, dge, H4, W + l.pool, l.Dp, TB, H4, l.Dp, W + l.wc_e, l.Dp));
    if (g->fc_mean_w && g->fc_lv_w && g->fc_lv_w == g->fc_mean_w + (size_t)Z * g->ld_fc_mean_w && g->ld_fc_lv_w == g->ld_fc_mean_w) {
      SSC_TRY(queue_dw(c, q, W + l.dmulv, 2 * Z, he_new, l.Hp, TB, 2 * Z, H, g->fc_mean_w, g->ld_fc_mean_w));
    } else {
      if (g->fc_mean_w) SSC_TRY(queue_dw(c, q, W + l.dmulv, 2 * Z, he_new, l.Hp, TB, Z, H, g->fc_mean_w, g->ld_fc_mean_w));
      if (g->fc_lv_w) SSC_TRY(queue_dw(c, q, W + l.dmulv + Z, 2 * Z, he_new, l.Hp, TB, Z, H, g->fc_lv_w, g->ld_fc_lv_w));
    }
    return SSC_OK;
  };
  auto queue_dec = [&](DwBatch& q) -> int {
    if (g->dec_w_ih) {
      float* gw = g->dec_w_ih; int ld = g->ld_dec_w_ih;
      SSC_TRY(queue_dw(c, q, dgd, H4, att, l.Fp, TB, H4, F, gw, ld));
      SSC_TRY(queue_dw(c, q, dgd, H4, h1_new, l.Hp, TB, H4, H, gw + F, ld));
      SSC_TRY(queue_dw(c, q, dgd, H4, hd_prev, l.Hp, TB, H4, H, gw + F + H, ld));
      if (l.Zp != Z) {
        SSC_TRY(queue_dw(c, q, dgd, H4, W + l.z, l.Zp, TB, H4, l.Zp, W + l.wz, l.Zp));
      } else {
        SSC_TRY(queue_dw(c, q, dgd, H4, W + l.z, l.Zp, TB, H4, Z, gw + zcol, ld));
      }
      if (l.D) SSC_TRY(queue_dw(c, q, dgd, H4, W + l.pool, l.Dp, TB, H4, l.Dp, W + l.wc_d, l.Dp));
    } else if (g->dec_w_hh) {
      SSC_TRY(queue_dw(c, q, dgd, H4, hd_prev, l.Hp, TB, H4, H, g->dec_w_hh, g->ld_dec_w_hh));
    }
    return SSC_OK;
  };
  if (one_flush) {
    SSC_TRY(queue_att(dwq));
    SSC_TRY(queue_enc(dwq));
    SSC_TRY(queue_dec(dwq));
    SSC_TRY(flush_dw(c, dwq));
  }
  if (phases & 128u) {
  if (!one_flush) {
    SSC_TRY(queue_att(dwq));
    SSC_TRY(flush_dw(c, dwq));
  }
  if (g->att_w_ih) {
    float* gw = g->att_w_ih; int ld = g->ld_att_w_ih;
    SSC_TRY(gemm(c, false, false, {{W + l.dga_sum, H4, W + l.avg, F, B}}, H4, F, gw + E, ld));
  }
  if (g->att_w_hh) {
    if (g->att_w_ih) {
      if (hipMemcpy2DAsync(g->att_w_hh, (size_t)g->ld_att_w_hh * sizeof(float), g->att_w_ih + E + F,
                           (size_t)g->ld_att_w_ih * sizeof(float), (size_t)H * sizeof(float), H4, hipMemcpyDeviceToDevice,
                           st) != hipSuccess)
        return SSC_EHIP;
    }
  }
  if (g->att_b_ih && g->att_b_hh) {
    SSC_TRY(ssc_colsum2(dga, H4, TB, H4, nullptr, g->att_b_ih, 1, g->att_b_hh, 0, c.slabs, st));
  } else {
    if (g->att_b_ih) SSC_TRY(ssc_colsum2(dga, H4, TB, H4, nullptr, g->att_b_ih, 1, nullptr, 0, c.slabs, st));
    if (g->att_b_hh) SSC_TRY(ssc_colsum2(dga, H4, TB, H4, nullptr, g->att_b_hh, 1, nullptr, 0, c.slabs, st));
  }
  if (g->wv) SSC_TRY(gemm(c, false, false, {{W + l.dpv, A, bt->feats, F, B * R}}, A, F, g->wv, g->ld_wv));
  if (g->wa) SSC_TRY(ssc_colsum(W + l.dwa, A, B, A, nullptr, g->wa, 1, 0, st));
  }
  if (phases & 4u) {
  if (!one_flush) {
    SSC_TRY(queue_enc(dwq));
    SSC_TRY(flush_dw(c, dwq));
  }
  if (g->enc_w_ih) {
    float* gw = g->enc_w_ih; int ld = g->ld_enc_w_ih;
    if (S == 1 && !l.D) SSC_TRY(ssc_colsum2(dge, H4, TB, H4, W + l.sent_all, gw + F + 2 * H, ld, nullptr, 0, c.slabs, st));
    if (l.D && hipMemcpy2DAsync(gw + F + 2 * H, (size_t)ld * sizeof(float), W + l.wc_e, (size_t)l.Dp * sizeof(float),
                                (size_t)l.SC * sizeof(float), H4, hipMemcpyDeviceToDevice, st) != hipSuccess)
      return SSC_EHIP;
  }
  if (g->enc_b_ih && g->enc_b_hh) {
    SSC_TRY(ssc_colsum2(dge, H4, TB, H4, nullptr, g->enc_b_ih, 1, g->enc_b_hh, 0, c.slabs, st));
  } else {
    if (g->enc_b_ih) SSC_TRY(ssc_colsum2(dge, H4, TB, H4, nullptr, g->enc_b_ih, 1, nullptr, 0, c.slabs, st));
    if (g->enc_b_hh) SSC_TRY(ssc_colsum2(dge, H4, TB, H4, nullptr, g->enc_b_hh, 1, nullptr, 0, c.slabs, st));
  }
  const float* dmulv = W + l.dmulv;
  if (g->fc_mean_b) SSC_TRY(ssc_colsum2(dmulv, 2 * Z, TB, Z, nullptr, g->fc_mean_b, 1, nullptr, 0, c.slabs, st));
  if (g->fc_lv_b) SSC_TRY(ssc_colsum2(dmulv + Z, 2 * Z, TB, Z, nullptr, g->fc_lv_b, 1, nullptr, 0, c.slabs, st));
  }
  if (phases & 8u) {
  if (!one_flush) {
    SSC_TRY(queue_dec(dwq));
    SSC_TRY(flush_dw(c, dwq));
  }
  if (g->dec_w_ih && l.Zp != Z) {
    if (hipMemcpy2DAsync(g->dec_w_ih + zcol, (size_t)g->ld_dec_w_ih * sizeof(float), W + l.wz, (size_t)l.Zp * sizeof(float),
                         (size_t)Z * sizeof(float), H4, hipMemcpyDeviceToDevice, st) != hipSuccess)
      return SSC_EHIP;
  }
  if (g->dec_w_ih) {
    float* gw = g->dec_w_ih; int ld = g->ld_dec_w_ih;
    if (S == 1 && !l.D) SSC_TRY(ssc_colsum2(dgd, H4, TB, H4, W + l.sent_all, gw + F + 2 * H, ld, nullptr, 0, c.slabs, st));
    if (l.D && hipMemcpy2DAsync(gw + F + 2 * H, (size_t)ld * sizeof(float), W + l.wc_d, (size_t)l.Dp * sizeof(float),
                                (size_t)l.SC * sizeof(float), H4, hipMemcpyDeviceToDevice, st) != hipSuccess)
      return SSC_EHIP;
  }
  if (g->dec_w_hh) {
    if (g->dec_w_ih) {
      if (hipMemcpy2DAsync(g->dec_w_hh, (size_t)g->ld_dec_w_hh * sizeof(float), g->dec_w_ih + F + H,
                           (size_t)g->ld_dec_w_ih * sizeof(float), (size_t)H * sizeof(float), H4, hipMemcpyDeviceToDevice,
                           st) != hipSuccess)
        return SSC_EHIP;
    }
  }
  if (g->dec_b_ih && g->dec_b_hh) {
    SSC_TRY(ssc_colsum2(dgd, H4, TB, H4, nullptr, g->dec_b_ih, 1, g->dec_b_hh, 0, c.slabs, st));
  } else {
    if (g->dec_b_ih) SSC_TRY(ssc_colsum2(dgd, H4, TB, H4, nullptr, g->dec_b_ih, 1, nullptr, 0, c.slabs, st));
    if (g->dec_b_hh) SSC_TRY(ssc_colsum2(dgd, H4, TB, H4, nullptr, g->dec_b_hh, 1, nullptr, 0, c.slabs, st));
  }
  }
  return SSC_OK;
}

extern "C" int ssc_train_bwd(const ssc_model_cfg* cfg, const ssc_params* p, const ssc_batch* bt, void* workspace,
                             size_t workspace_bytes, const float* gl, const float* gk, const ssc_params* g, void* stream) {
  return train_bwd_impl(cfg, p, bt, workspace, workspace_bytes, gl, gk, g, stream, 15u | 64u | 128u, 0.f, 0);
}

extern "C" int ssc_train_bwd_fb(const ssc_model_cfg* cfg, const ssc_params* p, const ssc_batch* bt, void* workspace,
                                size_t workspace_bytes, const float* gl, const float* gk, const ssc_params* g, float free_bits,
                                int free_bits_mode, void* stream) {
  return train_bwd_impl(cfg, p, bt, workspace, workspace_bytes, gl, gk, g, stream, 15u | 64u | 128u, free_bits, free_bits_mode);
}

extern "C" int ssc_train_bwd_phases(const ssc_model_cfg* cfg, const ssc_params* p, const ssc_batch* bt, void* workspace,
                                    size_t workspace_bytes, const float* gl, const float* gk, const ssc_params* g,
                                    unsigned phases, void* stream) {
  return ssc_train_bwd_phases_fb(cfg, p, bt, workspace, workspace_bytes, gl, gk, g, phases, 0.f, 0, stream);
}

extern "C" int ssc_train_bwd_phases_fb(const ssc_model_cfg* cfg, const ssc_params* p, const ssc_batch* bt, void* workspace,
                                       size_t workspace_bytes, const float* gl, const float* gk, const ssc_params* g,
                                       unsigned phases, float free_bits, int free_bits_mode, void* stream) {
  return ssc_train_bwd_phases_ss(cfg, p, bt, workspace, workspace_bytes, gl, gk, g, phases, free_bits, free_bits_mode, 0, stream);
}

extern "C" int ssc_train_bwd_ss(const ssc_model_cfg* cfg, const ssc_params* p, const ssc_batch* bt, void* workspace,
                                size_t workspace_bytes, const float* gl, const float* gk, const ssc_params* g, float free_bits,
                                int free_bits_mode, int fed_inputs, void* stream) {
  return train_bwd_impl(cfg, p, bt, workspace, workspace_bytes, gl, gk, g, stream, 15u | 64u | 128u, free_bits, free_bits_mode, fed_inputs);
}

extern "C" int ssc_train_bwd_phases_ss(const ssc_model_cfg* cfg, const ssc_params* p, const ssc_batch* bt, void* workspace,
                                       size_t workspace_bytes, const float* gl, const float* gk, const ssc_params* g,
                                       unsigned phases, float free_bits, int free_bits_mode, int fed_inputs, void* stream) {
  if (phases == 0 || phases > 255u) return SSC_EINVAL;
  if (phases & 2u) phases |= 64u | 128u;
  return train_bwd_impl(cfg, p, bt, workspace, workspace_bytes, gl, gk, g, stream, phases, free_bits, free_bits_mode, fed_inputs);
}
```

style-seqcvae_amd/ssc_runtime/lib.py:

```python
import ctypes as C
import os

_HERE = os.path.dirname(os.path.abspath(__file__))
DEBUG_ENV = os.environ.get("SSC_DEBUG", "") == "1"
LIB_PATH = (DEBUG_ENV and os.environ.get("SSC_LIB_PATH")) or os.path.join(os.path.dirname(_HERE), "libssc_hip.so")
SSC_MAX_SEG = 6

c_float_p = C.POINTER(C.c_float)
c_i64_p = C.POINTER(C.c_int64)
vp = C.c_void_p


class SscError(RuntimeError):
    CODES = {-1: "SSC_EINVAL", -2: "SSC_EALIGN", -3: "SSC_EHIP", -4: "SSC_EWORKSPACE"}

    def __init__(self, fn, rc, hip=0):
        super().__init__(f"{fn} failed: {self.CODES.get(rc, rc)}" + (f" (hipError {hip})" if rc == -3 else ""))
        self.rc = rc


class GemmSeg(C.Structure):
    _fields_ = [("A", vp), ("B", vp), ("lda", C.c_int), ("ldb", C.c_int), ("K", C.c_int),
                ("A16", vp), ("B16", vp), ("lda16", C.c_int), ("ldb16", C.c_int)]


class GemmDesc(C.Structure):
    _fields_ = [("seg", GemmSeg * SSC_MAX_SEG), ("nseg", C.c_int), ("M", C.c_int), ("N", C.c_int), ("a_kc", C.c_int),
                ("b_kc", C.c_int), ("C", vp), ("ldc", C.c_int), ("bias", vp), ("accumulate", C.c_int),
                ("splits", C.c_int), ("workspace", vp), ("workspace_floats", C.c_size_t), ("m_count", vp), ("a_rows", vp),
                ("c_rows", vp), ("k_count", vp), ("ka_rows", vp), ("kb_rows", vp), ("a_scale", vp), ("b_scale", vp), ("topk_part", vp)]


class LstmFwdDesc(C.Structure):
    _fields_ = [("B", C.c_int), ("H", C.c_int), ("slabs", vp), ("nslab", C.c_int), ("slab_stride", C.c_size_t),
                ("add0", vp), ("ld_add0", C.c_int), ("add1", vp), ("ld_add1", C.c_int), ("rows_per_add1", C.c_int),
                ("b_ih", vp), ("b_hh", vp), ("sent", vp), ("wcol", vp), ("ldwcol", C.c_int), ("c_prev", vp),
                ("ld_cprev", C.c_int), ("gates_out", vp), ("c_out", vp), ("ld_cout", C.c_int), ("h_out", vp),
                ("ld_hout", C.c_int), ("add0_rows", vp), ("slab_rows", vp), ("slabs2", vp), ("nslab2", C.c_int),
                ("slab2_stride", C.c_size_t), ("slab2_rows", vp), ("c_prev_rows", vp), ("rows", vp), ("row_count", vp),
                ("h_planes", vp), ("ld_hplanes", C.c_int), ("planes_scale", vp)]


class LstmBwdDesc(C.Structure):
    _fields_ = [("B", C.c_int), ("H", C.c_int), ("dh", vp), ("ld_dh", C.c_int), ("dh2", vp), ("ld_dh2", C.c_int),
                ("dc_in", vp), ("ld_dcin", C.c_int), ("gates", vp), ("c_prev", vp), ("ld_cprev", C.c_int),
                ("c_new", vp), ("ld_cnew", C.c_int), ("dG", vp), ("dc_prev", vp), ("ld_dcprev", C.c_int), ("dgsum", vp),
                ("slabsA", vp), ("nA", C.c_int), ("strideA", C.c_size_t), ("slabsB", vp), ("nB", C.c_int),
                ("strideB", C.c_size_t)]


class LatentFwdDesc(C.Structure):
    _fields_ = [("B", C.c_int), ("Z", C.c_int), ("mulv", vp), ("ldmulv", C.c_int), ("nslab", C.c_int),
                ("slab_stride", C.c_size_t), ("bmu", vp), ("blv", vp), ("eps", vp), ("ldeps", C.c_int),
                ("kld_mode", C.c_int), ("sent", vp), ("pm_scale", C.c_float), ("prior_var", C.c_float), ("w", vp),
                ("mu", vp), ("lv", vp), ("z", vp), ("ldz", C.c_int), ("kld_acc", vp), ("pm", vp), ("ldpm", C.c_int)]


class LatentBwdDesc(C.Structure):
    _fields_ = [("B", C.c_int), ("Z", C.c_int), ("dz", vp), ("lddz", C.c_int), ("eps", vp), ("ldeps", C.c_int),
                ("mu", vp), ("lv", vp), ("ldz", C.c_int), ("kld_mode", C.c_int), ("sent", vp), ("pm_scale", C.c_float),
                ("prior_var", C.c_float), ("w", vp), ("gk", vp), ("dmulv", vp), ("lddmulv", C.c_int),
                ("nslab", C.c_int), ("slab_stride", C.c_size_t), ("pm", vp), ("ldpm", C.c_int), ("dpm", vp), ("lddpm", C.c_int)]


class ModelCfg(C.Structure):
    _fields_ = [("V", C.c_int), ("E", C.c_int), ("H", C.c_int), ("A", C.c_int), ("F", C.c_int), ("Z", C.c_int),
                ("S", C.c_int), ("tied", C.c_int), ("kld_mode", C.c_int), ("pm_scale", C.c_float),
                ("prior_var", C.c_float), ("pad", C.c_int), ("boundary", C.c_int), ("gemm_mode", C.c_int),
                ("label_smoothing", C.c_float)]


class FreeBits(C.Structure):
    _fields_ = [("lambda_", C.c_float), ("mode", C.c_int), ("kld_raw", vp), ("gate_step", vp), ("dim_acc", vp), ("lddim", C.c_int),
                ("gate_dim", vp)]


PARAM_FIELDS = [("emb", True), ("att_w_ih", True), ("att_w_hh", True), ("att_b_ih", False), ("att_b_hh", False),
                ("wq", True), ("wv", True), ("wa", False), ("enc_w_ih", True), ("enc_w_hh", True), ("enc_b_ih", False),
                ("enc_b_hh", False), ("dec_w_ih", True), ("dec_w_hh", True), ("dec_b_ih", False), ("dec_b_hh", False),
                ("fc_mean_w", True), ("fc_mean_b", False), ("fc_lv_w", True), ("fc_lv_b", False), ("out_w", True),
                ("out_b", False), ("proj_w", True), ("proj_b", False)]


def _param_fields():
    f = []
    for name, has_ld in PARAM_FIELDS:
        f.append((name, vp))
        if has_ld:
            f.append(("ld_" + name, C.c_int))
    return f


class Params(C.Structure):
    _fields_ = _param_fields()


class Batch(C.Structure):
    _fields_ = [("B", C.c_int), ("R", C.c_int), ("L", C.c_int), ("feats", vp), ("caps", vp), ("sentiment", vp),
                ("eps", vp), ("obj_atts", vp)]


SSC_XGMI_MAX_RANKS = 8


class XgmiComm(C.Structure):
    _fields_ = [("world", C.c_int), ("rank", C.c_int), ("buf", vp * SSC_XGMI_MAX_RANKS), ("flags", vp * SSC_XGMI_MAX_RANKS)]


class DecodeStepDesc(C.Structure):
    _fields_ = [("G", C.c_int), ("R", C.c_int), ("rows_per_image", C.c_int), ("feats", vp), ("imgbuf", vp),
                ("tokens", vp), ("sentiment", vp), ("eps", vp), ("h1", vp), ("c1", vp), ("hd", vp), ("cd", vp),
                ("h1_out", vp), ("c1_out", vp), ("hd_out", vp), ("cd_out", vp), ("alpha", vp), ("log_probs", vp),
                ("raw_logits", C.c_int), ("emb_override", C.c_int), ("parent", vp), ("group", C.c_int), ("att_table", C.c_int),
# ... 24 lines not shown
class SamplerDesc(C.Structure):
    _fields_ = [("kind", C.c_int), ("top_k", C.c_int), ("top_p", C.c_float), ("temperature", C.c_float), ("seed", C.c_uint64)]


class SchedSampling(C.Structure):
    _fields_ = [("prob", C.c_float), ("sampler", SamplerDesc)]


class ScoreDesc(C.Structure):
    _fields_ = [("nimg", C.c_int), ("R", C.c_int), ("n_captions", C.c_int), ("n_samples", C.c_int), ("max_len", C.c_int),
                ("end_index", C.c_int), ("feats", vp), ("imgbuf", vp), ("sentiment", vp), ("obj_atts", vp), ("targets", vp),
                ("eps0", vp), ("eps", vp), ("log_probs", vp), ("token_lp", vp), ("token_rank", vp), ("n_tokens", vp)]


class PosteriorRowsDesc(C.Structure):
    _fields_ = [("T", C.c_int), ("B", C.c_int), ("Z", C.c_int), ("mu", vp), ("lv", vp), ("z", vp), ("ldz", C.c_int), ("eps", vp),
                ("ldeps", C.c_int), ("w", vp), ("pm", vp), ("ldpm", C.c_int), ("kld_mode", C.c_int), ("sent", vp),
                ("pm_scale", C.c_float), ("prior_var", C.c_float), ("log_ratio", vp), ("kl", vp), ("kl_dim", vp), ("ld", C.c_int),
                ("step_kl", vp), ("step_ratio", vp)]


class GumbelDesc(C.Structure):
    _fields_ = [("temperature", C.c_float), ("seed", C.c_uint64)]


class DiverseDesc(C.Structure):
    _fields_ = [("groups", C.c_int), ("strength", C.c_float)]


SSC_RULES_MAX_LEN = 64
SSC_RULES_MAX_SUPPRESS = 8


class RulesDesc(C.Structure):
    _fields_ = [("no_repeat_ngram", C.c_int), ("min_length", C.c_int), ("n_suppress", C.c_int),
                ("suppress", C.c_int * SSC_RULES_MAX_SUPPRESS), ("length_penalty", C.c_float * SSC_RULES_MAX_LEN)]


class RulesState(C.Structure):
    _fields_ = [("hist", vp), ("len", vp), ("hist_out", vp), ("len_out", vp), ("score_out", vp), ("ld_hist", C.c_int)]


class EvalRefs(C.Structure):
    _fields_ = [("I", C.c_int), ("nref", C.c_int), ("ntok", C.c_int), ("W", C.c_int), ("ref_offsets", vp), ("tok_offsets", vp),
                ("tokens", vp), ("style", vp), ("state", vp), ("state_bytes", C.c_size_t)]


class EvalScoreDesc(C.Structure):
    _fields_ = [("predictions", vp), ("P", C.c_int), ("N", C.c_int), ("steps", C.c_int), ("boundary_index", C.c_int), ("V", C.c_int),
                ("id_map", vp), ("style_ids", vp), ("ref_image", vp), ("scores", vp), ("counts", vp), ("image_counts", vp), ("top5", vp)]


class EvalSetDesc(C.Structure):
    _fields_ = [("predictions", vp), ("P", C.c_int), ("N", C.c_int), ("steps", C.c_int), ("boundary_index", C.c_int), ("V", C.c_int),
                ("id_map", vp), ("ref_image", vp), ("set_counts", vp), ("kernel", vp), ("eigenvalues", vp), ("distinct", vp)]


class EvalConsensusDesc(C.Structure):
    _fields_ = [("predictions", vp), ("P", C.c_int), ("N", C.c_int), ("steps", C.c_int), ("boundary_index", C.c_int), ("V", C.c_int),
                ("id_map", vp), ("neighbours", vp), ("k", C.c_int), ("scores", vp), ("pool_refs", vp), ("pick", vp), ("order", vp)]


class ScstDesc(C.Structure):
    _fields_ = [("P", C.c_int), ("N", C.c_int), ("steps", C.c_int), ("L", C.c_int), ("end_index", C.c_int), ("predictions", vp),
                ("scores", vp), ("base_scores", vp), ("reward_weights", C.c_double * 6), ("baseline", C.c_int),
                ("loss_scale", C.c_double), ("kld_scale", C.c_double), ("caps", vp), ("lengths", vp), ("reward", vp),
                ("advantage", vp), ("gl", vp), ("gk", vp), ("stats", vp)]


_i, _f, _sz = C.c_int, C.c_float, C.c_size_t
SYMBOLS = {
    "ssc_version": (_i, []),
    "ssc_last_hip_error": (_i, []),
    "ssc_arch": (C.c_char_p, []),
    "ssc_gemm": (_i, [C.POINTER(GemmDesc), vp]),
    "ssc_gemm_dw_group": (_i, [C.POINTER(C.POINTER(GemmDesc)), _i, vp]),
    "ssc_gemm_auto_splits": (_i, [_i, _i, _i]),
    "ssc_pow2_scale": (_i, [vp, _sz, _i, _sz, _i, vp, _i, vp, vp]),
    "ssc_split_f16": (_i, [vp, _i, _i, _i, vp, vp, _i, vp, vp, vp]),
    "ssc_decode_planes_ld": (_i, [vp]),
    "ssc_set_gemm_mode": (_i, [_i]),
    "ssc_feat_prep": (_i, [vp, _i, _i, _i, vp, vp, vp]),
    "ssc_prep_tokens": (_i, [vp, _i, _i, _i, _i, vp, vp, vp, vp]),
    "ssc_embed_gather": (_i, [vp, _i, vp, _i, _i, vp, _i, vp]),
    "ssc_embed_scatter_add": (_i, [vp, _i, vp, _i, _i, vp, _i, _i, vp]),
    "ssc_lstm_fwd": (_i, [C.POINTER(LstmFwdDesc), vp]),
    "ssc_lstm_fwd_z": (_i, [C.POINTER(LstmFwdDesc), vp, _i, vp, _i, _i, vp]),
    "ssc_lstm_fwd_p": (_i, [C.POINTER(LstmFwdDesc), vp, _i, _i, vp, vp]),
    "ssc_lstm_fwd_img": (_i, [C.POINTER(LstmFwdDesc), vp, _i, vp, _i, _i, vp]),
    "ssc_lstm_bwd_x": (_i, [C.POINTER(LstmBwdDesc), vp, _i, vp, _i, _i, vp]),
    "ssc_lstm_bwd": (_i, [C.POINTER(LstmBwdDesc), vp]),
    "ssc_attn_logits": (_i, [vp, _i, vp, vp, _i, _i, _i, _i, vp, vp]),
    "ssc_attn_fwd": (_i, [vp, _i, vp, vp, vp, vp, _i, _i, _i, _i, _i, vp, vp, vp, _i, vp]),
    "ssc_attn_weights": (_i, [vp, _i, vp, vp, vp, _i, _i, _i, _i, vp, vp, vp]),
    "ssc_attn_pool": (_i, [vp, vp, _i, _i, _i, _i, vp, _i, vp]),
    "ssc_attn_fwd_pool": (_i, [vp, _i, vp, vp, vp, vp, _i, _i, _i, _i, _i, vp, vp, vp, _i, vp, _i, vp, _i, vp]),
    "ssc_attn_bwd_pool": (_i, [vp, _i, vp, _i, vp, vp, vp, vp, _i, _i, _i, _i, vp, _i, vp, vp, vp, vp, _i, vp, _i, _i, vp, _i, vp]),
    "ssc_attn_bwd": (_i, [vp, _i, vp, _i, vp, vp, vp, vp, _i, _i, _i, _i, vp, _i, vp, vp, vp, vp]),
    "ssc_latent_fwd": (_i, [C.POINTER(LatentFwdDesc), vp]),
    "ssc_latent_prior_sample": (_i, [vp, _i, vp, _f, _f, _i, _i, vp, _i, vp]),
    "ssc_latent_prior_sample_pm": (_i, [vp, _i, vp, _i, vp, _i, vp, _f, _f, _i, _i, vp, _i, vp]),
    "ssc_latent_bwd": (_i, [C.POINTER(LatentBwdDesc), vp]),
    "ssc_latent_fwd_fb": (_i, [C.POINTER(LatentFwdDesc), C.POINTER(FreeBits), vp]),
    "ssc_latent_bwd_fb": (_i, [C.POINTER(LatentBwdDesc), C.POINTER(FreeBits), vp]),
    "ssc_latent_fb_finish": (_i, [vp, _i, _i, _i, _f, vp, vp, vp, vp]),
    "ssc_ce_fwd": (_i, [vp, _i, vp, vp, vp, _i, _i, _i, vp, vp, vp]),
    "ssc_ce_bwd": (_i, [vp, _i, vp, vp, vp, vp, vp, _i, _i, _i, vp]),
    "ssc_ce_fwd_smooth": (_i, [vp, _i, vp, vp, vp, _i, _i, _i, _f, vp, vp, vp, vp]),
    "ssc_ce_bwd_smooth": (_i, [vp, _i, vp, vp, vp, vp, vp, _i, _i, _i, _f, vp]),
    "ssc_log_softmax": (_i, [vp, _i, _i, _i, vp, _i, vp]),
    "ssc_colsum": (_i, [vp, _i, _i, _i, vp, vp, _i, _i, vp]),
    "ssc_colsum2": (_i, [vp, _i, _i, _i, vp, vp, _i, vp, _i, vp, vp]),
    "ssc_copy_strided": (_i, [vp, _sz, _i, vp, vp]),
    "ssc_bias_tanh": (_i, [vp, _i, _i, _i, vp, vp]),
    "ssc_tanh_bwd": (_i, [vp, _i, vp, _i, _i, _i, vp]),
    "ssc_fill": (_i, [vp, _sz, _f, vp]),
    "ssc_sq_norm": (_i, [vp, _sz, vp, vp, vp]),
    "ssc_sgd_step": (_i, [vp, vp, vp, _sz, vp, _f, _f, _f, _f, _f, _i, vp]),
    "ssc_adam_step": (_i, [vp, vp, vp, vp, _sz, vp, _f, _f, _f, _f, _f, _f, _f, _i, _i, vp]),
    "ssc_train_workspace_bytes": (_sz, [C.POINTER(ModelCfg), _i, _i, _i]),
    "ssc_train_fwd": (_i, [C.POINTER(ModelCfg), C.POINTER(Params), C.POINTER(Batch), vp, _sz, vp, vp, vp]),
    "ssc_train_bwd": (_i, [C.POINTER(ModelCfg), C.POINTER(Params), C.POINTER(Batch), vp, _sz, vp, vp, C.POINTER(Params), vp]),
    "ssc_train_bwd_phases": (_i, [C.POINTER(ModelCfg), C.POINTER(Params), C.POINTER(Batch), vp, _sz, vp, vp, C.POINTER(Params),
                                  C.c_uint, vp]),
    "ssc_train_workspace_view": (vp, [C.POINTER(ModelCfg), _i, _i, _i, vp, _i, C.POINTER(C.c_int)]),
    "ssc_train_fwd_fb": (_i, [C.POINTER(ModelCfg), C.POINTER(Params), C.POINTER(Batch), vp, _sz, vp, vp, _f, _i, vp]),
    "ssc_train_bwd_fb": (_i, [C.POINTER(ModelCfg), C.POINTER(Params), C.POINTER(Batch), vp, _sz, vp, vp, C.POINTER(Params), _f, _i, vp]),
    "ssc_train_bwd_phases_fb": (_i, [C.POINTER(ModelCfg), C.POINTER(Params), C.POINTER(Batch), vp, _sz, vp, vp, C.POINTER(Params),
                                     C.c_uint, _f, _i, vp]),
    "ssc_train_free_bits_view": (vp, [C.POINTER(ModelCfg), _i, _i, _i, vp, _i, C.POINTER(C.c_int)]),
    "ssc_xgmi_enable_peer": (_i, [_i]),
    "ssc_xgmi_ipc_export": (_i, [vp, vp, C.POINTER(C.c_size_t)]),
    "ssc_xgmi_ipc_open": (_i, [vp, C.POINTER(vp)]),
    "ssc_xgmi_ipc_close": (_i, [vp]),
    "ssc_xgmi_peek": (_i, [vp, vp, _sz]),
    "ssc_xgmi_allreduce": (_i, [C.POINTER(XgmiComm), _sz, _sz, C.c_uint, C.c_uint, vp, vp]),
    "ssc_decode_image_bytes": (_sz, [C.POINTER(ModelCfg), _i, _i]),
    "ssc_decode_prepare": (_i, [C.POINTER(ModelCfg), C.POINTER(Params), vp, _i, _i, vp, _sz, vp]),
    "ssc_decode_prepare_from": (_i, [C.POINTER(ModelCfg), C.POINTER(Params), vp, _i, _i, vp, _sz, vp, _i, _i, vp]),
    "ssc_decode_step_workspace_bytes": (_sz, [C.POINTER(ModelCfg), _i, _i]),
    "ssc_decode_step": (_i, [C.POINTER(ModelCfg), C.POINTER(Params), C.POINTER(DecodeStepDesc), vp, _sz, vp]),
    "ssc_decode_ungathered_ok": (_i, [C.POINTER(ModelCfg), _i, _i, _i, _i]),
    "ssc_beam_first": (_i, [vp, _i, vp, _i, _i, _i, _i, vp, vp, vp]),
    "ssc_beam_step": (_i, [vp, _i, vp, vp, vp, _i, _i, _i, _i, _i, _i, vp, vp, vp, vp, vp, vp]),
    "ssc_beam_first_logits": (_i, [vp, _i, vp, _i, _i, _i, _i, vp, vp, vp]),
    "ssc_beam_step_logits": (_i, [vp, _i, vp, vp, vp, _i, _i, _i, _i, _i, _i, vp, vp, vp, vp, vp, vp]),
    "ssc_gather_rows": (_i, [vp, _i, vp, _i, _i, _i, vp, vp]),
    "ssc_beam_backtrace": (_i, [vp, vp, _i, _i, _i, vp, vp]),
    "ssc_fsm_tables_bytes": (_sz, [C.POINTER(FsmDims)]),
    "ssc_fsm_compile": (_i, [vp, C.POINTER(FsmDims), vp, _sz, vp]),
    "ssc_beam_first_fsm": (_i, [C.POINTER(BeamDesc), vp]),
    "ssc_beam_step_fsm": (_i, [C.POINTER(BeamDesc), vp]),
    "ssc_beam_step_parts": (_i, [C.POINTER(BeamDesc), vp, vp]),
    "ssc_beam_backtrace_ctl": (_i, [vp, vp, vp, _i, _i, _i, _i, vp, vp]),
    "ssc_host_device_ptr": (_i, [vp, C.POINTER(vp)]),
    "ssc_decode_search_workspace_bytes": (_sz, [C.POINTER(ModelCfg), C.POINTER(SearchDesc)]),
    "ssc_decode_search": (_i, [C.POINTER(ModelCfg), C.POINTER(Params), C.POINTER(SearchDesc), vp, _sz, vp]),
    "ssc_sample_rows": (_i, [vp, _i, _i, _i, C.POINTER(SamplerDesc), vp, _i, vp, vp, _i, vp, vp, vp, vp]),
    "ssc_decode_sample_workspace_bytes": (_sz, [C.POINTER(ModelCfg), C.POINTER(SearchDesc)]),
    "ssc_decode_sample": (_i, [C.POINTER(ModelCfg), C.POINTER(Params), C.POINTER(SearchDesc), C.POINTER(SamplerDesc), vp, _sz, vp]),
    "ssc_sched_mix_rows": (_i, [vp, _i, _i, _i, vp, vp, vp, vp, _i, _i, _i, C.POINTER(SchedSampling), vp, vp, vp, _i, vp]),
    "ssc_train_fwd_ss": (_i, [C.POINTER(ModelCfg), C.POINTER(Params), C.POINTER(Batch), vp, _sz, vp, vp, _f, _i, C.POINTER(SchedSampling),
                              vp]),
    "ssc_train_sched_view": (vp, [C.POINTER(ModelCfg), _i, _i, _i, vp, _i, C.POINTER(C.c_int)]),
    "ssc_train_bwd_ss": (_i, [C.POINTER(ModelCfg), C.POINTER(Params), C.POINTER(Batch), vp, _sz, vp, vp, C.POINTER(Params), _f, _i, _i, vp]),
    "ssc_train_bwd_phases_ss": (_i, [C.POINTER(ModelCfg), C.POINTER(Params), C.POINTER(Batch), vp, _sz, vp, vp, C.POINTER(Params),
# ... 98 lines not shown
```

Baseline: 7992 captions/s.

## Fuse prep kernels, dual-store weight gradients, and fold small dW GEMM into group

```diff
diff --git a/include/ssc.h b/include/ssc.h
--- a/include/ssc.h
+++ b/include/ssc.h
@@ -41,6 +41,7 @@
   const int* k_count; const int* ka_rows; const int* kb_rows;
   const float* a_scale; const float* b_scale;
   float* topk_part;
+  float* C2; int ldc2;
 } ssc_gemm_desc;
 
 int ssc_pow2_scale(const float* x, size_t rows, int cols, size_t ld, int target_log2, float* out, int combine, float* scratch,
@@ -60,6 +61,9 @@
 
 int ssc_prep_tokens(const int64_t* caps, int B, int L, int pad, int boundary, int64_t* tokens_tm, float* w_tm,
                     float* nvalid, void* stream);
+
+int ssc_prep_tokens_rows(const int64_t* caps, int B, int L, int pad, int boundary, int64_t* tokens_tm, float* w_tm,
+                         float* nvalid, int* act, int* live, int* ident, void* stream);
 
 int ssc_embed_gather(const float* table, int ldt, const int64_t* ids, int n, int E, float* out, int ldo, void* stream);
 int ssc_embed_scatter_add(float* dtable, int ldt, const int64_t* ids, int n, int E, const float* d, int ldd, int pad,
diff --git a/style-seqcvae_amd/csrc/gemm.hip b/style-seqcvae_amd/csrc/gemm.hip
--- a/style-seqcvae_amd/csrc/gemm.hip
+++ b/style-seqcvae_amd/csrc/gemm.hip
@@ -1,6 +1,8 @@
 #include <stdio.h>
 #include <stdlib.h>
 #include <string.h>
+
+#include <type_traits>
 
 #include "ssc_common.h"
 #include "ssc_debug.h"
@@ -932,6 +934,7 @@
 template <int TM, int TN> constexpr int x3w_lds_bytes() { return 2 * 3 * (X3wPlane<TM>::BYTES + X3wPlane<TN>::BYTES) + X3W_STAMP_BYTES; }
 template <int TM, int TN> constexpr int x3w_lds_bytes_f16() { return 2 * 2 * (X3wPlane<TM>::BYTES + X3wPlane<TN>::BYTES) + X3W_STAMP_BYTES; }
 
+struct KTnArgs;
 template <bool A_KC, bool B_KC, bool KG, int TM, int TN, int PF, int NPW, bool F16 = false, class Args = KArgs>
 __device__ __forceinline__ void x3w_body(const Args& a, const int blk_x, const int blk_y, const int blk_z, const int grid_x,
                                          const int grid_y, const int grid_z, const int thr) {
@@ -1424,11 +1427,27 @@
         } else {
           *reinterpret_cast<float4*>(dst) = v;
         }
+        if constexpr (std::is_same_v<Args, KTnArgs>) {
+          if (a.out2) {
+            float* dst2 = a.out2 + (size_t)grow * a.ldo2 + gcol;
+            if (!(a.ldo2 & 3) && !(reinterpret_cast<uintptr_t>(a.out2) & 15)) {
+              *reinterpret_cast<float4*>(dst2) = v;
+            } else {
+              dst2[0] = v.x; dst2[1] = v.y; dst2[2] = v.z; dst2[3] = v.w;
+            }
+          }
+        }
       } else {
         const float e[4] = {v.x, v.y, v.z, v.w};
 #pragma unroll
         for (int q = 0; q < 4; ++q) {
-          if (gcol + q < a.N) dst[q] = e[q] + (a.bias ? a.bias[gcol + q] : 0.f) + (a.accumulate ? dst[q] : 0.f);
+          if (gcol + q < a.N) {
+            const float r = e[q] + (a.bias ? a.bias[gcol + q] : 0.f) + (a.accumulate ? dst[q] : 0.f);
+            dst[q] = r;
+            if constexpr (std::is_same_v<Args, KTnArgs>) {
+              if (a.out2) a.out2[(size_t)grow * a.ldo2 + gcol + q] = r;
+            }
+          }
         }
       }
     }
@@ -1476,6 +1495,8 @@
   const int* kbrows;
   int lda, ldb, ldc, M, N, K, accumulate;
   int first;
+  float* C2;
+  int ldc2;
 };
 struct KTnList {
   KTnMember m[SSC_DW_MAX];
@@ -1498,6 +1519,8 @@
   int tile_gm, store_wt, member;
   float* topk;
   const float *a_scale, *b_scale;
+  float* out2;
+  int ldo2;
 };
 template <int PF, int NPW>
 __global__ __launch_bounds__(256 + 64 * NPW, 1) void gemm_x3w_kernel_tn_list(const KTnList g) {
@@ -1520,6 +1543,7 @@
     a.kcount = m.kcount; a.karows = m.karows; a.kbrows = m.kbrows;
     a.tile_gm = g.tile_gm; a.store_wt = g.store_wt; a.member = p;
     a.topk = nullptr; a.a_scale = a.b_scale = nullptr;
+    a.out2 = m.C2; a.ldo2 = m.ldc2;
     const int gx = (m.N + 127) / 128, gy = (m.M + 127) / 128;
     const int local = t - m.first;
     x3w_body<false, false, true, 128, 128, PF, NPW>(a, local % gx, local / gx, 0, gx, gy, 1, thr);
@@ -2070,6 +2094,7 @@
     m.kcount = di->k_count; m.karows = di->ka_rows; m.kbrows = di->kb_rows;
     m.lda = di->seg[0].lda; m.ldb = di->seg[0].ldb; m.ldc = di->ldc;
     m.M = di->M; m.N = di->N; m.K = di->seg[0].K; m.accumulate = di->accumulate;
+    m.C2 = di->C2; m.ldc2 = di->ldc2;
     m.first = first;
     first += ssc_cdiv(di->M, 128) * ssc_cdiv(di->N, 128);
     MN += (long)di->M * di->N;
@@ -2100,6 +2125,7 @@
     const ssc_gemm_desc* dj = d[j];
     KArgs& k = ka[j];
     SSC_TRY(build_args(dj, k));
+    if (dj->C2 && (dj->ldc2 < dj->N || !dj->C)) return SSC_EINVAL;
     const bool kg = k.karows || k.kbrows;
     const bool ok = x3w_ok(dj, k, num) && k.nseg == 1 && !dj->a_kc && !dj->b_kc && dj->C && dj->ldc >= dj->N && !k.mcount &&
                     !k.arows && !k.crows && (kg ? (k.kcount && k.karows && k.kbrows && !dj->bias) : !k.kcount);
@@ -2140,10 +2166,17 @@
       SSC_TRY(launch_x3w(x3w_big(false, false, false), g, false, false, "128x128 TN group", rec, st));
       i += m;
     } else {
-      SSC_TRY(ssc_gemm(d[i], (void*)st));
+      ssc_gemm_desc one = *d[i];
+      one.C2 = nullptr;
+      SSC_TRY(ssc_gemm(&one, (void*)st));
       ++i;
     }
   }
+  for (int j = 0; j < n; ++j)
+    if (d[j]->C2 && cls[j] != 2 &&
+        hipMemcpy2DAsync(d[j]->C2, (size_t)d[j]->ldc2 * sizeof(float), d[j]->C, (size_t)d[j]->ldc * sizeof(float),
+                         (size_t)d[j]->N * sizeof(float), d[j]->M, hipMemcpyDeviceToDevice, st) != hipSuccess)
+      return SSC_EHIP;
   return SSC_OK;
 }
 
@@ -2190,6 +2223,7 @@
   hipStream_t st = (hipStream_t)stream;
   KArgs k;
   SSC_TRY(build_args(d, k));
+  if (d->C2) return SSC_EINVAL;
   if (d->topk_part) {
     k.out = nullptr; k.ldo = d->N; k.slab_stride = 0; k.bias = d->bias; k.accumulate = 0;
     return launch(d, k, 1, st);
diff --git a/style-seqcvae_amd/csrc/pointwise.hip b/style-seqcvae_amd/csrc/pointwise.hip
--- a/style-seqcvae_amd/csrc/pointwise.hip
+++ b/style-seqcvae_amd/csrc/pointwise.hip
@@ -10,31 +10,48 @@
 
 namespace {
 
-__global__ void feat_mask_kernel(const float* __restrict__ feats, int BR, int F, float* __restrict__ mask) {
-  int row = blockIdx.x * (blockDim.x >> 6) + (threadIdx.x >> 6);
-  int lane = threadIdx.x & 63;
-  if (row >= BR) return;
-  const float* p = feats + (size_t)row * F;
-  float s = 0.f;
-  for (int f = lane; f < F; f += 64) s += fabsf(p[f]);
-  s = ssc_wave_sum(s);
-  if (lane == 0) mask[row] = s > 0.f ? 1.f : 0.f;
-}
-
-__global__ void feat_avg_kernel(const float* __restrict__ feats, const float* __restrict__ mask, int R, int F,
-                                float* __restrict__ avg) {
-  int b = blockIdx.y;
-  int f = blockIdx.x * blockDim.x + threadIdx.x;
-  if (f >= F) return;
-  const float* p = feats + (size_t)b * R * F + f;
-  const float* m = mask + (size_t)b * R;
-  float s = 0.f, n = 0.f;
-  for (int r = 0; r < R; ++r) {
-    float mr = m[r];
-    s += mr * p[(size_t)r * F];
-    n += mr;
-  }
-  avg[(size_t)b * F + f] = s / fmaxf(n, 1e-8f);
+constexpr int kFeatPrepThreads = 1024;
+__global__ __launch_bounds__(kFeatPrepThreads) void feat_prep_kernel(const float* __restrict__ feats, int R, int F,
+                                                                     float* __restrict__ mask, float* avg) {
+  extern __shared__ int nz[];
+  __shared__ float wave_n[kFeatPrepThreads / 64];
+  const int b = blockIdx.x, tid = threadIdx.x, lane = tid & 63;
+  const float* p = feats + (size_t)b * R * F;
+  for (int r = tid; r < R; r += kFeatPrepThreads) nz[r] = 0;
+  __syncthreads();
+  for (int f0 = 0; f0 < F; f0 += kFeatPrepThreads) {
+    const int f = f0 + tid;
+    const bool in = f < F;
+    const int fc = in ? f : F - 1;
+    float s = 0.f;
+    for (int r = 0; r < R; r += 8) {
+      float x[8];
+#pragma unroll
+      for (int u = 0; u < 8; ++u) x[u] = p[(size_t)min(r + u, R - 1) * F + fc];
+#pragma unroll
+      for (int u = 0; u < 8; ++u)
+        if (r + u < R) {
+          s += x[u];
+          const bool any = __ballot(in && fabsf(x[u]) > 0.f) != 0ull;
+          if (any && lane == 0) nz[r + u] = 1;
+        }
+    }
+    if (in) avg[(size_t)b * F + f] = s;
+  }
+  __syncthreads();
+  float n = 0.f;
+  for (int r = tid; r < R; r += kFeatPrepThreads) {
+    const float m = nz[r] ? 1.f : 0.f;
+    mask[(size_t)b * R + r] = m;
+    n += m;
+  }
+  n = ssc_wave_sum(n);
+  if (lane == 0) wave_n[tid >> 6] = n;
+  __syncthreads();
+  n = 0.f;
+  for (int q = 0; q < kFeatPrepThreads / 64; ++q) n += wave_n[q];
+  const float d = fmaxf(n, 1e-8f);
+  for (int f = tid; f < F; f += kFeatPrepThreads) avg[(size_t)b * F + f] = avg[(size_t)b * F + f] / d;
 }
 
 __global__ void prep_tokens_kernel(const int64_t* __restrict__ caps, int B, int L, int pad, int boundary,
@@ -702,9 +719,17 @@
   int n = blockIdx.x * blockDim.x + threadIdx.x;
   if (n >= N) return;
   float s = 0.f;
-  for (int r = 0; r < rows; ++r) {
-    float x = X[(size_t)r * ldx + n];
-    s += wrow ? wrow[r] * x : x;
+  for (int r = 0; r < rows; r += 8) {
+    float x[8];
+#pragma unroll
+    for (int u = 0; u < 8; ++u) {
+      const int rr = min(r + u, rows - 1);
+      x[u] = X[(size_t)rr * ldx + n];
+      if (wrow) x[u] = wrow[rr] * x[u];
+    }
+#pragma unroll
+    for (int u = 0; u < 8; ++u)
+      if (r + u < rows) s += x[u];
   }
   float* o = out + (size_t)n * out_stride;
   *o = accumulate ? *o + s : s;
@@ -849,10 +874,8 @@
 
 extern "C" int ssc_feat_prep(const float* feats, int B, int R, int F, float* mask, float* avg, void* stream) {
   if (!feats || !mask || !avg || B <= 0 || R <= 0 || F <= 0) return SSC_EINVAL;
-  int BR = B * R;
-  SSC_LAUNCH(feat_mask_kernel, dim3(ssc_cdiv(BR, 4)), dim3(256), 0, S(stream), feats, BR, F, mask);
-  SSC_CHECK_LAUNCH();
-  SSC_LAUNCH(feat_avg_kernel, dim3(ssc_cdiv(F, 256), B), dim3(256), 0, S(stream), feats, mask, R, F, avg);
+  if ((size_t)R * sizeof(int) > 48 * 1024) return SSC_EINVAL;
+  SSC_LAUNCH(feat_prep_kernel, dim3(B), dim3(kFeatPrepThreads), (size_t)R * sizeof(int), S(stream), feats, R, F, mask, avg);
   SSC_CHECK_LAUNCH();
   return SSC_OK;
 }
diff --git a/style-seqcvae_amd/csrc/sequence.hip b/style-seqcvae_amd/csrc/sequence.hip
--- a/style-seqcvae_amd/csrc/sequence.hip
+++ b/style-seqcvae_amd/csrc/sequence.hip
@@ -1,3 +1,4 @@
+#include <climits>
 #include <cstdlib>
 #include <initializer_list>
 
@@ -23,6 +24,7 @@
   size_t slabs, slab_floats, logits, lse, proj;
   size_t nllw0, nll;
   size_t kld_raw, fb_kdim, fb_gdim, fb_gstep, fb_acc;
+  size_t ident;
   size_t fed_ids, fed;
   size_t sl_q, sl_mulv, sl_gh1, sl_ghd, sl_ghd2, sl_ghe, sl_dqw, sl_dhe, sl_dz, small_floats, wsum_att, wsum_dec, wz;
   size_t sl_ga, sl_ge, sl_gd, gate_floats;
@@ -114,6 +116,7 @@
   l.fb_acc = l.take((size_t)B * l.Zp);
   l.fed_ids = l.take(2 * TB);
   l.fed = l.take(TB);
+  l.ident = l.take((size_t)B + 4);
   return l;
 }
 
@@ -178,14 +181,17 @@
   ssc_gemm_desc d[MAX];
   int n = 0;
 };
-int queue_dw(const Ctx& c, DwBatch& q, const float* A, int lda, const float* Bm, int ldb, int K, int M, int N, float* C, int ldc) {
+int queue_dw(const Ctx& c, DwBatch& q, const float* A, int lda, const float* Bm, int ldb, int K, int M, int N, float* C, int ldc,
+             const int* klist = nullptr, float* C2 = nullptr, int ldc2 = 0) {
   if (q.n >= DwBatch::MAX) return SSC_EINVAL;
   ssc_gemm_desc& d = q.d[q.n++];
   fill_desc(d, false, false, {{A, lda, Bm, ldb, K}}, M, N);
   d.C = C; d.ldc = ldc;
+  d.C2 = C2; d.ldc2 = ldc2;
   d.splits = 0;
   d.workspace = c.slabs; d.workspace_floats = c.slab_floats;
-  if (c.live_rows) { d.k_count = c.live_count; d.ka_rows = c.live_rows; d.kb_rows = c.live_rows; }
+  if (klist) { d.k_count = klist; d.ka_rows = klist + 4; d.kb_rows = klist + 4; }
+  else if (c.live_rows) { d.k_count = c.live_count; d.ka_rows = c.live_rows; d.kb_rows = c.live_rows; }
   return SSC_OK;
 }
 int flush_dw(const Ctx& c, DwBatch& q) {
@@ -205,16 +211,13 @@
   q.n = 0;
   return rc;
 }
-__global__ __launch_bounds__(1024) void build_active_rows_kernel(const float* __restrict__ w, int n, int B, int* __restrict__ act,
-                                                                 int* __restrict__ live) {
-  __shared__ int part[1024];
+template <class WT>
+__device__ __forceinline__ void ordered_row_list(WT wt, bool suffix, int n, int B, int* __restrict__ out, int* part) {
   const int tid = threadIdx.x;
-  const bool suffix = blockIdx.x == 1;
-  int* out = suffix ? live : act;
   auto flag = [&](int i) -> bool {
-    if (!suffix) return w[i] != 0.f;
+    if (!suffix) return wt(i);
     for (int r = i; r < n; r += B)
-      if (w[r] != 0.f) return true;
+      if (wt(r)) return true;
     return false;
   };
   const int per = (n + 1023) / 1024;
@@ -234,6 +237,49 @@
     if (flag(i)) out[4 + pos++] = i;
   if (tid == 1023) out[0] = part[1023];
   for (int i = part[1023] + tid; i < n; i += 1024) out[4 + i] = 0;
+}
+__device__ __forceinline__ void identity_row_list(int B, int* __restrict__ out) {
+  if (threadIdx.x == 0) out[0] = B;
+  for (int i = threadIdx.x; i < B; i += blockDim.x) out[4 + i] = i;
+}
+__global__ __launch_bounds__(1024) void build_active_rows_kernel(const float* __restrict__ w, int n, int B, int* __restrict__ act,
+                                                                 int* __restrict__ live, int* __restrict__ ident) {
+  __shared__ int part[1024];
+  if (blockIdx.x == 2) { identity_row_list(B, ident); return; }
+  const bool suffix = blockIdx.x == 1;
+  ordered_row_list([&](int i) { return w[i] != 0.f; }, suffix, n, B, suffix ? live : act, part);
+}
+constexpr int kPrepRowsMaxLds = 60 * 1024;
+__global__ __launch_bounds__(1024) void prep_tokens_rows_kernel(const int64_t* __restrict__ caps, int B, int L, int pad, int boundary,
+                                                                int64_t* __restrict__ tok, float* __restrict__ w,
+                                                                float* __restrict__ nvalid, int* __restrict__ act,
+                                                                int* __restrict__ live, int* __restrict__ ident) {
+  extern __shared__ unsigned char wsh[];
+  __shared__ int part[1024];
+  if (blockIdx.x == 2) { identity_row_list(B, ident); return; }
+  const int n = (L + 1) * B;
+  const bool first = blockIdx.x == 0;
+  for (int i = threadIdx.x; i < n; i += 1024) {
+    const int t = i / B, b = i - t * B;
+    const int64_t* cb = caps + (size_t)b * L;
+    int nb = 0;
+    for (int j = 0; j < L; ++j) nb += cb[j] != pad;
+    auto token = [&](int tt) -> int64_t { return tt == nb ? (int64_t)boundary : tt < L ? cb[tt] : (int64_t)0; };
+    const int64_t tk = token(t);
+    const bool on = tk != pad;
+    wsh[i] = on;
+    if (!first) continue;
+    tok[(size_t)(t + 1) * B + b] = tk;
+    w[i] = on ? 1.f : 0.f;
+    if (t == 0) {
+      tok[b] = boundary;
+      float nv = 0.f;
+      for (int tt = 0; tt <= L; ++tt) nv += token(tt) != pad ? 1.f : 0.f;
+      nvalid[b] = nv;
+    }
+  }
+  __syncthreads();
+  ordered_row_list([&](int i) { return wsh[i] != 0; }, !first, n, B, first ? act : live, part);
 }
 
 int gemm_to_slabs(const Ctx& c, float* region, size_t cap, bool a_kc, bool b_kc, std::initializer_list<Seg> segs, int M,
@@ -361,6 +407,24 @@
   if (g_loop.bwd) {
     if (hipEventSynchronize(g_loop.e[3]) != hipSuccess || hipEventElapsedTime(bwd_loop_ms, g_loop.e[2], g_loop.e[3]) != hipSuccess) return SSC_EHIP;
   }
+  return SSC_OK;
+}
+
+extern "C" int ssc_prep_tokens_rows(const int64_t* caps, int B, int L, int pad, int boundary, int64_t* tokens_tm, float* w_tm,
+                                    float* nvalid, int* act, int* live, int* ident, void* stream) {
+  if (!caps || !tokens_tm || !w_tm || !nvalid || !act || !live || B <= 0 || L <= 0) return SSC_EINVAL;
+  hipStream_t st = (hipStream_t)stream;
+  const size_t n = (size_t)(L + 1) * B;
+  if (n > (size_t)INT_MAX) return SSC_EINVAL;
+  if (n <= (size_t)kPrepRowsMaxLds) {
+    SSC_LAUNCH(prep_tokens_rows_kernel, dim3(ident ? 3 : 2), dim3(1024), n, st, caps, B, L, pad, boundary, tokens_tm, w_tm, nvalid,
+               act, live, ident);
+    SSC_CHECK_LAUNCH();
+    return SSC_OK;
+  }
+  SSC_TRY(ssc_prep_tokens(caps, B, L, pad, boundary, tokens_tm, w_tm, nvalid, stream));
+  SSC_LAUNCH(build_active_rows_kernel, dim3(ident ? 3 : 2), dim3(1024), 0, st, w_tm, (int)n, B, act, live, ident);
+  SSC_CHECK_LAUNCH();
   return SSC_OK;
 }
 
@@ -447,11 +511,9 @@
   const size_t sH = (size_t)B * l.Hp;
   const bool fb_on = free_bits > 0.f;
 
-  SSC_TRY(ssc_prep_tokens(bt->caps, B, l.L, cfg->pad, cfg->boundary, tok, W + l.w, W + l.nvalid, st));
   int* act = (int*)(W + l.act);
   int* live = (int*)(W + l.live);
-  SSC_LAUNCH(build_active_rows_kernel, dim3(2), dim3(1024), 0, st, W + l.w, TB, B, act, live);
-  SSC_CHECK_LAUNCH();
+  SSC_TRY(ssc_prep_tokens_rows(bt->caps, B, l.L, cfg->pad, cfg->boundary, tok, W + l.w, W + l.nvalid, act, live, (int*)(W + l.ident), st));
   c.act_count = act; c.act_rows = act + 4;
   c.live_count = live; c.live_rows = live + 4;
   SSC_TRY(ssc_feat_prep(bt->feats, B, R, F, W + l.mask, W + l.avg, st));
@@ -965,8 +1027,9 @@
     if (g->att_w_ih) {
       float* gw = g->att_w_ih; int ld = g->ld_att_w_ih;
       SSC_TRY(queue_dw(c, q, dga, H4, W + l.emb, l.Ep, TB, H4, E, gw, ld));
-      SSC_TRY(queue_dw(c, q, dga, H4, h1_prev, l.Hp, TB, H4, H, gw + E + F, ld));
+      SSC_TRY(queue_dw(c, q, dga, H4, h1_prev, l.Hp, TB, H4, H, gw + E + F, ld, nullptr, g->att_w_hh, g->ld_att_w_hh));
       SSC_TRY(queue_dw(c, q, dga, H4, hd_prev, l.Hp, TB, H4, H, gw + E + F + H, ld));
+      SSC_TRY(queue_dw(c, q, W + l.dga_sum, H4, W + l.avg, F, B, H4, F, gw + E, ld, (const int*)(W + l.ident)));
     } else if (g->att_w_hh) {
       SSC_TRY(queue_dw(c, q, dga, H4, h1_prev, l.Hp, TB, H4, H, g->att_w_hh, g->ld_att_w_hh));
     }
@@ -995,7 +1058,7 @@
       float* gw = g->dec_w_ih; int ld = g->ld_dec_w_ih;
       SSC_TRY(queue_dw(c, q, dgd, H4, att, l.Fp, TB, H4, F, gw, ld));
       SSC_TRY(queue_dw(c, q, dgd, H4, h1_new, l.Hp, TB, H4, H, gw + F, ld));
-      SSC_TRY(queue_dw(c, q, dgd, H4, hd_prev, l.Hp, TB, H4, H, gw + F + H, ld));
+      SSC_TRY(queue_dw(c, q, dgd, H4, hd_prev, l.Hp, TB, H4, H, gw + F + H, ld, nullptr, g->dec_w_hh, g->ld_dec_w_hh));
       if (l.Zp != Z) {
         SSC_TRY(queue_dw(c, q, dgd, H4, W + l.z, l.Zp, TB, H4, l.Zp, W + l.wz, l.Zp));
       } else {
@@ -1018,18 +1081,6 @@
     SSC_TRY(queue_att(dwq));
     SSC_TRY(flush_dw(c, dwq));
   }
-  if (g->att_w_ih) {
-    float* gw = g->att_w_ih; int ld = g->ld_att_w_ih;
-    SSC_TRY(gemm(c, false, false, {{W + l.dga_sum, H4, W + l.avg, F, B}}, H4, F, gw + E, ld));
-  }
-  if (g->att_w_hh) {
-    if (g->att_w_ih) {
-      if (hipMemcpy2DAsync(g->att_w_hh, (size_t)g->ld_att_w_hh * sizeof(float), g->att_w_ih + E + F,
-                           (size_t)g->ld_att_w_ih * sizeof(float), (size_t)H * sizeof(float), H4, hipMemcpyDeviceToDevice,
-                           st) != hipSuccess)
-        return SSC_EHIP;
-    }
-  }
   if (g->att_b_ih && g->att_b_hh) {
     SSC_TRY(ssc_colsum2(dga, H4, TB, H4, nullptr, g->att_b_ih, 1, g->att_b_hh, 0, c.slabs, st));
   } else {
@@ -1058,8 +1109,12 @@
     if (g->enc_b_hh) SSC_TRY(ssc_colsum2(dge, H4, TB, H4, nullptr, g->enc_b_hh, 1, nullptr, 0, c.slabs, st));
   }
   const float* dmulv = W + l.dmulv;
-  if (g->fc_mean_b) SSC_TRY(ssc_colsum2(dmulv, 2 * Z, TB, Z, nullptr, g->fc_mean_b, 1, nullptr, 0, c.slabs, st));
-  if (g->fc_lv_b) SSC_TRY(ssc_colsum2(dmulv + Z, 2 * Z, TB, Z, nullptr, g->fc_lv_b, 1, nullptr, 0, c.slabs, st));
+  if (g->fc_mean_b && g->fc_lv_b == g->fc_mean_b + Z) {
+    SSC_TRY(ssc_colsum2(dmulv, 2 * Z, TB, 2 * Z, nullptr, g->fc_mean_b, 1, nullptr, 0, c.slabs, st));
+  } else {
+    if (g->fc_mean_b) SSC_TRY(ssc_colsum2(dmulv, 2 * Z, TB, Z, nullptr, g->fc_mean_b, 1, nullptr, 0, c.slabs, st));
+    if (g->fc_lv_b) SSC_TRY(ssc_colsum2(dmulv + Z, 2 * Z, TB, Z, nullptr, g->fc_lv_b, 1, nullptr, 0, c.slabs, st));
+  }
   }
   if (phases & 8u) {
   if (!one_flush) {
@@ -1078,14 +1133,6 @@
                                 (size_t)l.SC * sizeof(float), H4, hipMemcpyDeviceToDevice, st) != hipSuccess)
       return SSC_EHIP;
   }
-  if (g->dec_w_hh) {
-    if (g->dec_w_ih) {
-      if (hipMemcpy2DAsync(g->dec_w_hh, (size_t)g->ld_dec_w_hh * sizeof(float), g->dec_w_ih + F + H,
-                           (size_t)g->ld_dec_w_ih * sizeof(float), (size_t)H * sizeof(float), H4, hipMemcpyDeviceToDevice,
-                           st) != hipSuccess)
-        return SSC_EHIP;
-    }
-  }
   if (g->dec_b_ih && g->dec_b_hh) {
     SSC_TRY(ssc_colsum2(dgd, H4, TB, H4, nullptr, g->dec_b_ih, 1, g->dec_b_hh, 0, c.slabs, st));
   } else {
diff --git a/style-seqcvae_amd/ssc_runtime/lib.py b/style-seqcvae_amd/ssc_runtime/lib.py
--- a/style-seqcvae_amd/ssc_runtime/lib.py
+++ b/style-seqcvae_amd/ssc_runtime/lib.py
@@ -28,7 +28,8 @@
     _fields_ = [("seg", GemmSeg * SSC_MAX_SEG), ("nseg", C.c_int), ("M", C.c_int), ("N", C.c_int), ("a_kc", C.c_int),
                 ("b_kc", C.c_int), ("C", vp), ("ldc", C.c_int), ("bias", vp), ("accumulate", C.c_int),
                 ("splits", C.c_int), ("workspace", vp), ("workspace_floats", C.c_size_t), ("m_count", vp), ("a_rows", vp),
-                ("c_rows", vp), ("k_count", vp), ("ka_rows", vp), ("kb_rows", vp), ("a_scale", vp), ("b_scale", vp), ("topk_part", vp)]
+                ("c_rows", vp), ("k_count", vp), ("ka_rows", vp), ("kb_rows", vp), ("a_scale", vp), ("b_scale", vp), ("topk_part", vp),
+                ("C2", vp), ("ldc2", C.c_int)]
 
 
 class LstmFwdDesc(C.Structure):
@@ -219,6 +220,7 @@
     "ssc_set_gemm_mode": (_i, [_i]),
     "ssc_feat_prep": (_i, [vp, _i, _i, _i, vp, vp, vp]),
     "ssc_prep_tokens": (_i, [vp, _i, _i, _i, _i, vp, vp, vp, vp]),
+    "ssc_prep_tokens_rows": (_i, [vp, _i, _i, _i, _i, vp, vp, vp, vp, vp, vp, vp]),
     "ssc_embed_gather": (_i, [vp, _i, vp, _i, _i, vp, _i, vp]),
     "ssc_embed_scatter_add": (_i, [vp, _i, vp, _i, _i, vp, _i, _i, vp]),
     "ssc_lstm_fwd": (_i, [C.POINTER(LstmFwdDesc), vp]),
```

Measured after the change: 8083 captions/s (median of 6 runs). +1.1%, better.
